# starreeze/drin

Measured on AMD Instinct MI355X. Metric: mention x candidate pairs scored/sec, higher is better.
Workload: dtype bf16x3; 1 GPU; wikimel-shaped scoring forward: 100-cand (+1 answer slot), D=768, R=2048, L=128, P=49, T=64 token-level entity text; parallelism=dp1 (mentions sharded, no collective)

## Files before the change

### drin_amd/_lib.py

```python
from __future__ import annotations

import ctypes as C
import os
from typing import Optional

_HERE = os.path.dirname(os.path.abspath(__file__))
LIB_PATH = os.environ.get("DRIN_LIB_PATH") or os.path.join(_HERE, "libdrin_hip.so")
MAX_LAYERS = 8
ABI_VERSION = 12

OK, E_SHAPE, E_NULL, E_ALIGN, E_WORKSPACE, E_HIP, E_UNSUPPORTED, E_INDEX = 0, -1, -2, -3, -4, -5, -6, -7
PREC_F32, PREC_BF16X3, PREC_BF16X3_ALL, PREC_BF16X3_IF16 = 0, 1, 3, 5
ROW_ACT = {"none": 0, "relu": 1, "gelu": 2}
FEAT_F32, FEAT_BF16 = 0, 1
CACHE_F32, CACHE_MIXED_F16 = 0, 1
CACHE_FORMATS = {"f32": CACHE_F32, "mixed_f16": CACHE_MIXED_F16}
ACTIVATIONS = {"gelu": 1, "sigmoid": 2, "relu": 3, "tanh": 4, "silu": 5}

fp = C.POINTER(C.c_float)
ip = C.POINTER(C.c_int64)


class DrinConfigC(C.Structure):
    _fields_ = [
        ("batch", C.c_int32), ("num_candidates", C.c_int32), ("embed_dim", C.c_int32), ("image_dim", C.c_int32),
        ("mention_tokens", C.c_int32), ("image_regions", C.c_int32), ("mention_objects", C.c_int32),
        ("entity_objects", C.c_int32), ("entity_tokens", C.c_int32), ("mention_object_inner", C.c_int32),
        ("entity_image_inner", C.c_int32), ("entity_object_inner", C.c_int32), ("num_layers", C.c_int32),
        ("dynamic_edges", C.c_int32), ("edge_enabled", C.c_float * 4), ("layer_norm_eps", C.c_float),
        ("cosine_eps", C.c_float), ("miei_eps", C.c_float), ("clip_scale", C.c_float), ("precision", C.c_int32),
        ("num_entities", C.c_int32), ("vector_edges", C.c_int32), ("feature_dtype", C.c_int32),
        ("vertex_activation", C.c_int32), ("edge_activation", C.c_int32), ("cache_format", C.c_int32),
    ]


class DrinBatchC(C.Structure):
    _fields_ = [
        ("mention_text", C.c_void_p), ("mention_start", C.c_void_p), ("mention_end", C.c_void_p),
        ("mention_image", C.c_void_p), ("mention_object", C.c_void_p), ("mention_object_score", C.c_void_p),
        ("entity_text", C.c_void_p), ("entity_text_mask", C.c_void_p), ("entity_image", C.c_void_p),
        ("entity_object", C.c_void_p), ("entity_object_score", C.c_void_p), ("miet_similarity", C.c_void_p),
        ("mtei_similarity", C.c_void_p), ("entity_index", C.c_void_p), ("entity_text_cls", C.c_void_p),
        ("index_status", C.c_void_p),
    ]


class DrinLayerParamsC(C.Structure):
    _fields_ = [(n, C.c_void_p) for n in ("w_h", "b_h", "w_u", "b_u", "w_v", "b_v", "ln_weight", "ln_bias", "w_m", "b_m")]


class DrinParamsC(C.Structure):
    _fields_ = [(n, C.c_void_p) for n in (
        "w_mention_text", "b_mention_text", "w_entity_text", "b_entity_text",
        "w_mention_image", "b_mention_image", "w_entity_image", "b_entity_image")] + [("layer", DrinLayerParamsC * MAX_LAYERS)]


class DrinParamGradsC(C.Structure):
    _fields_ = DrinParamsC._fields_


class DrinInputGradsC(C.Structure):
    _fields_ = [(n, C.c_void_p) for n in (
        "mention_text", "mention_image", "mention_object", "mention_object_score", "entity_text", "entity_text_cls",
        "entity_image", "entity_object", "entity_object_score", "miet_similarity", "mtei_similarity", "scratch")] + [
        ("scratch_bytes", C.c_size_t)]


class DrinMelhiConfigC(C.Structure):
    _fields_ = [("batch", C.c_int32), ("num_candidates", C.c_int32), ("embed_dim", C.c_int32), ("image_dim", C.c_int32),
                ("mention_tokens", C.c_int32), ("image_regions", C.c_int32), ("precision", C.c_int32),
                ("cosine_eps", C.c_float), ("thres_tmim", C.c_float), ("thres_imie", C.c_float)]


class DrinMelhiBatchC(C.Structure):
    _fields_ = [(n, C.c_void_p) for n in (
        "mention_feature", "mention_mask", "start", "end", "mention_image", "entity_feature", "entity_image")]


MELHI_PARAMS = ("w_image_map_text", "b_image_map_text", "w_ih", "w_hh", "b_ih", "b_hh", "w_mention_final_map",
                "b_mention_final_map", "w_entity_final_map", "b_entity_final_map")


class DrinMelhiParamsC(C.Structure):
    _fields_ = [(n, C.c_void_p) for n in MELHI_PARAMS]


class DrinMelhiParamGradsC(C.Structure):
    _fields_ = DrinMelhiParamsC._fields_


class DrinGhmfcConfigC(C.Structure):
    _fields_ = [("batch", C.c_int32), ("num_candidates", C.c_int32), ("embed_dim", C.c_int32), ("image_dim", C.c_int32),
                ("mention_tokens", C.c_int32), ("image_regions", C.c_int32), ("num_heads", C.c_int32),
                ("entity_tokens", C.c_int32), ("precision", C.c_int32), ("layer_norm_eps", C.c_float), ("cosine_eps", C.c_float)]


class DrinGhmfcBatchC(C.Structure):
    _fields_ = [(n, C.c_void_p) for n in ("mention_feature", "mention_mask", "mention_image", "entity_feature", "entity_mask")]


GHMFC_CROSS_PARAMS = ("a2b_wq", "a2b_wk", "a2b_wv", "a2b_in_bias", "a2b_wo", "a2b_bo", "a2b_ffn_w", "a2b_ffn_b", "b2a_in_w",
                      "b2a_in_bias", "b2a_wo", "b2a_bo", "b2a_ffn_w", "b2a_ffn_b", "ln0_w", "ln0_b", "ln1_w", "ln1_b", "ln2_w",
                      "ln2_b", "ln3_w", "ln3_b")


class DrinGhmfcCrossParamsC(C.Structure):
    _fields_ = [(n, C.c_void_p) for n in GHMFC_CROSS_PARAMS]


class DrinGhmfcParamsC(C.Structure):
    _fields_ = [("t2v", DrinGhmfcCrossParamsC), ("v2t", DrinGhmfcCrossParamsC)] + [(n, C.c_void_p) for n in (
        "w_text_linear", "b_text_linear", "w_image_linear", "b_image_linear", "w_score_linear", "b_score_linear", "w_entity",
        "b_entity")]


class DrinGemmRouteC(C.Structure):
    _fields_ = [(n, C.c_int32) for n in ("launches", "family", "bm", "bn", "w_planes", "a_lo", "f16", "persist", "indexed", "accumulate",
                                         "ksplit", "splits")] + [(n, C.c_int64) for n in ("tiles", "whole_tiles", "tile0", "work_items")]


class DrinGemmProbeArgsC(C.Structure):
    _fields_ = [("struct_size", C.c_size_t), ("op", C.c_int32), ("precision", C.c_int32), ("accumulate", C.c_int32),
                ("row_tile_wgs", C.c_int32), ("row_tile_begin", C.c_int64), ("row_tile_end", C.c_int64), ("a", C.c_void_p),
                ("a_lo", C.c_void_p), ("lda", C.c_int64), ("b", C.c_void_p), ("b_hi", C.c_void_p), ("b_lo", C.c_void_p),
                ("ldb", C.c_int64), ("bias", C.c_void_p), ("y", C.c_void_p), ("ldy", C.c_int64), ("rows", C.c_int64),
                ("n_out", C.c_int32), ("k", C.c_int32), ("scratch", C.c_void_p), ("scratch_floats", C.c_size_t),
                ("a_index", C.c_void_p), ("row_scale", C.c_void_p), ("b_scale", C.c_void_p), ("route", DrinGemmRouteC)]


class DrinWgradProductC(C.Structure):
    _fields_ = [("dy", C.c_void_p), ("lddy", C.c_int64), ("x", C.c_void_p), ("ldx", C.c_int64), ("x_index", C.c_void_p), ("dw", C.c_void_p),
                ("lddw", C.c_int64), ("db", C.c_void_p), ("rows", C.c_int64), ("n_out", C.c_int32), ("k", C.c_int32)]


class DrinWgradProductRouteC(C.Structure):
    _fields_ = [(n, C.c_int32) for n in ("kernel", "slices", "in_place", "db_rode", "db_slices", "launch")] + [("rows_per_slice", C.c_int64)]


WGRAD_PROBE_MAX, WGRAD_ROUTE_LAUNCHES = 16, 8


class DrinWgradRouteC(C.Structure):
    _fields_ = [(n, C.c_int32) for n in ("gemm_launches", "colsum_launches", "sum_launches", "reduce_launches", "sum_dsts", "sum_segs",
                                         "nn_family", "nn_bm", "nn_bn", "nn_splits", "nn_wt_form", "nn_accumulate")] + [
        ("grid", C.c_int64 * WGRAD_ROUTE_LAUNCHES), ("product", DrinWgradProductRouteC * WGRAD_PROBE_MAX)]


class DrinWgradProbeArgsC(C.Structure):
    _fields_ = [("struct_size", C.c_size_t), ("op", C.c_int32), ("precision", C.c_int32), ("staged", C.c_int32), ("n_products", C.c_int32),
                ("layers_done_after", C.c_int32), ("accumulate", C.c_int32), ("wt_form", C.c_int32), ("reserved", C.c_int32),
                ("scratch", C.c_void_p), ("scratch_floats", C.c_size_t), ("wt", C.c_void_p), ("wt_floats", C.c_size_t),
                ("product", DrinWgradProductC * WGRAD_PROBE_MAX), ("route", DrinWgradRouteC)]


WGRAD_TN_GROUP, WGRAD_TN_F32_GROUP, WGRAD_TN, WGRAD_COLSUM_BATCH, WGRAD_PASS, WGRAD_NN = range(1, 7)
WGRAD_KERNEL = {0: "none", 1: "tn_bf16x3", 2: "tn_f32_small", 3: "tn_f32_large"}
WGRAD_WT_NONE, WGRAD_WT_F32_SCRATCH, WGRAD_WT_PLANES = range(3)
PROBE_GEMM_NT, PROBE_GEMM_NT_BF16X3, PROBE_GEMM_NT_BF16X3_P4, PROBE_GEMM_X3_PLANES, PROBE_GEMM_F16_PLANES, PROBE_TO_F16_SCALED = range(1, 7)
GEMM_FAMILY = {0: "none", 1: "bf16x3", 2: "bf16x3_p4", 3: "planes", 4: "planes_p4", 5: "f32", 6: "f32_gemv"}


class DrinTraceC(C.Structure):
    _fields_ = [(n, C.c_void_p * (MAX_LAYERS + 1)) for n in (
        "mention_text_vertex", "mention_image_vertex", "entity_text_vertex", "entity_image_vertex", "edges")]


EXPORTS = {
    "drin_version": (C.c_int, []),
    "drin_last_error": (C.c_char_p, []),
    "drin_build_info": (C.c_char_p, []),
    "drin_default_config": (C.c_int, [C.POINTER(DrinConfigC)]),
    "drin_host_selftest": (C.c_int, []),
    "drin_workspace_bytes": (C.c_size_t, [C.POINTER(DrinConfigC), C.c_int]),
    "drin_edges_fwd": (C.c_int, [C.POINTER(DrinConfigC), C.POINTER(DrinBatchC), C.c_void_p, C.c_void_p, C.c_void_p]),
    "drin_pool_fwd": (C.c_int, [C.POINTER(DrinConfigC), C.POINTER(DrinBatchC), C.c_void_p, C.c_void_p, C.c_void_p, C.c_void_p]),
    "drin_linear_fwd": (C.c_int, [C.c_void_p, C.c_void_p, C.c_void_p, C.c_void_p, C.c_int64, C.c_int32, C.c_int32, C.c_int32, C.c_void_p]),
    "drin_linear_bwd": (C.c_int, [C.c_void_p, C.c_void_p, C.c_void_p, C.c_void_p, C.c_void_p, C.c_void_p, C.c_int64, C.c_int32,
                                  C.c_int32, C.c_int32, C.c_void_p, C.c_size_t, C.c_void_p]),
    "drin_forward": (C.c_int, [C.POINTER(DrinConfigC), C.POINTER(DrinBatchC), C.POINTER(DrinParamsC), C.c_void_p,
                               C.c_size_t, C.c_void_p, C.c_int, C.POINTER(DrinTraceC), C.c_void_p]),
    "drin_forward_staged": (C.c_int, [C.POINTER(DrinConfigC), C.POINTER(DrinBatchC), C.POINTER(DrinParamsC), C.c_void_p,
                                      C.c_size_t, C.c_void_p, C.c_int, C.POINTER(DrinTraceC), C.c_void_p, C.c_void_p]),
    "drin_backward": (C.c_int, [C.POINTER(DrinConfigC), C.POINTER(DrinBatchC), C.POINTER(DrinParamsC), C.c_void_p,
                                C.c_size_t, C.c_void_p, C.POINTER(DrinParamGradsC), C.c_void_p]),
    "drin_backward_staged": (C.c_int, [C.POINTER(DrinConfigC), C.POINTER(DrinBatchC), C.POINTER(DrinParamsC), C.c_void_p,
                                       C.c_size_t, C.c_void_p, C.POINTER(DrinParamGradsC), C.c_void_p, C.c_void_p]),
    "drin_backward_ex": (C.c_int, [C.POINTER(DrinConfigC), C.POINTER(DrinBatchC), C.POINTER(DrinParamsC), C.c_void_p,
                                   C.c_size_t, C.c_void_p, C.POINTER(DrinParamGradsC), C.POINTER(DrinInputGradsC), C.c_void_p,
                                   C.c_void_p]),
    "drin_input_grad_scratch_bytes": (C.c_size_t, [C.POINTER(DrinConfigC)]),
    "drin_pool_bwd": (C.c_int, [C.POINTER(DrinConfigC), C.c_void_p, C.c_void_p, C.c_void_p, C.c_void_p, C.c_void_p]),
    "drin_fused_supported": (C.c_int, [C.POINTER(DrinConfigC)]),
    "drin_indexed_supported": (C.c_int, [C.POINTER(DrinConfigC)]),
    "drin_prepared_bytes": (C.c_size_t, [C.POINTER(DrinConfigC)]),
    "drin_fused_workspace_bytes": (C.c_size_t, [C.POINTER(DrinConfigC)]),
    "drin_workgroups_per_mention": (C.c_int32, [C.POINTER(DrinConfigC), C.c_int32]),
    "drin_index_status": (C.c_int, [C.c_void_p, C.c_void_p]),
    "drin_image_contraction_passes": (C.c_int32, [C.POINTER(DrinConfigC), C.c_int32]),
    "drin_image_contraction_side_tiles": (C.c_int32, [C.POINTER(DrinConfigC), C.c_int32]),
    "drin_prepare": (C.c_int, [C.POINTER(DrinConfigC), C.POINTER(DrinParamsC), C.c_void_p, C.c_size_t, C.c_void_p]),
    "drin_forward_prepared": (C.c_int, [C.POINTER(DrinConfigC), C.POINTER(DrinBatchC), C.POINTER(DrinParamsC), C.c_void_p,
                                        C.c_void_p, C.c_size_t, C.c_void_p, C.c_void_p]),
    "drin_entity_cache_bytes": (C.c_size_t, [C.POINTER(DrinConfigC)]),
    "drin_entity_cache_build_workspace_bytes": (C.c_size_t, [C.POINTER(DrinConfigC)]),
    "drin_cached_workspace_bytes": (C.c_size_t, [C.POINTER(DrinConfigC)]),
    "drin_build_entity_cache": (C.c_int, [C.POINTER(DrinConfigC), C.POINTER(DrinBatchC), C.POINTER(DrinParamsC), C.c_void_p,
                                          C.c_void_p, C.c_size_t, C.c_void_p, C.c_size_t, C.c_void_p]),
    "drin_forward_cached": (C.c_int, [C.POINTER(DrinConfigC), C.POINTER(DrinBatchC), C.POINTER(DrinParamsC), C.c_void_p,
                                      C.c_void_p, C.c_void_p, C.c_size_t, C.c_void_p, C.c_void_p]),
    "drin_split_planes": (C.c_int, [C.c_void_p, C.c_void_p, C.c_void_p, C.c_int64, C.c_void_p]),
    "drin_linear_planes_fwd": (C.c_int, [C.c_void_p, C.c_void_p, C.c_void_p, C.c_void_p, C.c_void_p, C.c_void_p,
                                         C.c_int64, C.c_int32, C.c_int32, C.c_void_p]),
    "drin_gemm_probe": (C.c_int, [C.POINTER(DrinGemmProbeArgsC), C.c_void_p]),
    "drin_wgrad_probe": (C.c_int, [C.POINTER(DrinWgradProbeArgsC), C.c_void_p]),
    "drin_loss_workspace_bytes": (C.c_size_t, [C.c_int32]),
    "drin_triplet_topk": (C.c_int, [C.c_void_p, C.c_void_p, C.c_int32, C.c_int32, C.c_float, C.POINTER(C.c_int32), C.c_int32,
                                    C.c_void_p, C.c_void_p, C.c_void_p, C.c_void_p, C.c_size_t, C.c_void_p]),
    "drin_adam_step": (C.c_int, [C.c_void_p, C.c_void_p, C.c_void_p, C.c_void_p, C.c_int64, C.c_float, C.c_float, C.c_float,
                                 C.c_float, C.c_float, C.c_float, C.c_void_p]),
    "drin_melhi_workspace_bytes": (C.c_size_t, [C.POINTER(DrinMelhiConfigC), C.c_int]),
    "drin_melhi_forward": (C.c_int, [C.POINTER(DrinMelhiConfigC), C.POINTER(DrinMelhiBatchC), C.POINTER(DrinMelhiParamsC), C.c_void_p,
                                     C.c_void_p, C.c_void_p, C.c_size_t, C.c_void_p, C.c_void_p]),
    "drin_melhi_backward": (C.c_int, [C.POINTER(DrinMelhiConfigC), C.POINTER(DrinMelhiBatchC), C.POINTER(DrinMelhiParamsC),
                                      C.c_void_p, C.c_void_p, C.c_void_p, C.c_size_t, C.c_void_p, C.POINTER(DrinMelhiParamGradsC),
                                      C.c_void_p]),
    "drin_ghmfc_workspace_bytes": (C.c_size_t, [C.POINTER(DrinGhmfcConfigC)]),
    "drin_ghmfc_forward": (C.c_int, [C.POINTER(DrinGhmfcConfigC), C.POINTER(DrinGhmfcBatchC), C.POINTER(DrinGhmfcParamsC), C.c_void_p,
                                     C.c_size_t, C.c_void_p, C.c_void_p, C.c_void_p]),
    "drin_attention": (C.c_int, [C.c_void_p, C.c_int64, C.c_void_p, C.c_int64, C.c_void_p, C.c_int64, C.c_void_p, C.c_void_p, C.c_int64,
                                 C.c_int32, C.c_int32, C.c_int32, C.c_int32, C.c_int32, C.c_void_p]),
    "drin_attention_train_fwd": (C.c_int, [C.c_void_p, C.c_int64, C.c_void_p, C.c_int64, C.c_void_p, C.c_int64, C.c_void_p, C.c_void_p,
                                           C.c_int64, C.c_void_p, C.c_int32, C.c_int32, C.c_int32, C.c_int32, C.c_int32, C.c_void_p]),
    "drin_attention_bwd": (C.c_int, [C.c_void_p, C.c_int64, C.c_void_p, C.c_int64, C.c_void_p, C.c_int64, C.c_void_p, C.c_void_p,
                                     C.c_int64, C.c_void_p, C.c_void_p, C.c_int64, C.c_void_p, C.c_int64, C.c_void_p, C.c_int64,
                                     C.c_void_p, C.c_int64, C.c_void_p, C.c_int32, C.c_int32, C.c_int32, C.c_int32, C.c_int32,
                                     C.c_void_p]),
    "drin_attention_dropout_fwd": (C.c_int, [C.c_void_p, C.c_int64, C.c_void_p, C.c_int64, C.c_void_p, C.c_int64, C.c_void_p, C.c_void_p,
                                             C.c_int64, C.c_void_p, C.c_int32, C.c_int32, C.c_int32, C.c_int32, C.c_int32, C.c_float,
                                             C.c_uint64, C.c_uint64, C.c_void_p]),
    "drin_attention_dropout_bwd": (C.c_int, [C.c_void_p, C.c_int64, C.c_void_p, C.c_int64, C.c_void_p, C.c_int64, C.c_void_p, C.c_void_p,
                                             C.c_int64, C.c_void_p, C.c_void_p, C.c_int64, C.c_void_p, C.c_int64, C.c_void_p, C.c_int64,
                                             C.c_void_p, C.c_int64, C.c_void_p, C.c_int32, C.c_int32, C.c_int32, C.c_int32, C.c_int32,
                                             C.c_float, C.c_uint64, C.c_uint64, C.c_void_p]),
    "drin_attention_dropout_keep": (C.c_int, [C.c_uint64, C.c_uint64, C.c_int32, C.c_int32, C.c_int32, C.c_int32, C.c_float, C.c_void_p]),
    "drin_attention_mfma_fwd": (C.c_int, [C.c_void_p, C.c_int64, C.c_void_p, C.c_int64, C.c_void_p, C.c_int64, C.c_void_p, C.c_void_p,
                                          C.c_int64, C.c_void_p, C.c_int32, C.c_int32, C.c_int32, C.c_int32, C.c_int32, C.c_float,
                                          C.c_uint64, C.c_uint64, C.c_void_p]),
    "drin_attention_mfma_bwd": (C.c_int, [C.c_void_p, C.c_int64, C.c_void_p, C.c_int64, C.c_void_p, C.c_int64, C.c_void_p, C.c_void_p,
                                          C.c_int64, C.c_void_p, C.c_void_p, C.c_int64, C.c_void_p, C.c_int64, C.c_void_p, C.c_int64,
                                          C.c_void_p, C.c_int64, C.c_void_p, C.c_int32, C.c_int32, C.c_int32, C.c_int32, C.c_int32,
                                          C.c_float, C.c_uint64, C.c_uint64, C.c_void_p]),
    "drin_layernorm_res_train_fwd": (C.c_int, [C.c_void_p, C.c_void_p, C.c_void_p, C.c_void_p, C.c_void_p, C.c_void_p, C.c_void_p,
                                               C.c_int64, C.c_int32, C.c_float, C.c_void_p]),
    "drin_layernorm_res_bwd_scratch_floats": (C.c_size_t, [C.c_int64, C.c_int32]),
    "drin_layernorm_res_bwd": (C.c_int, [C.c_void_p, C.c_void_p, C.c_void_p, C.c_void_p, C.c_void_p, C.c_void_p, C.c_void_p, C.c_void_p,
                                         C.c_void_p, C.c_void_p, C.c_size_t, C.c_int64, C.c_int32, C.c_void_p]),
    "drin_seq_max_train_fwd": (C.c_int, [C.c_void_p, C.c_void_p, C.c_void_p, C.c_int32, C.c_int32, C.c_int32, C.c_void_p]),
    "drin_seq_max_bwd": (C.c_int, [C.c_void_p, C.c_void_p, C.c_void_p, C.c_int32, C.c_int32, C.c_int32, C.c_void_p]),
    "drin_gate_mix_fwd": (C.c_int, [C.c_void_p, C.c_void_p, C.c_void_p, C.c_void_p, C.c_void_p, C.c_int32, C.c_int32, C.c_void_p]),
    "drin_gate_mix_bwd_scratch_floats": (C.c_size_t, [C.c_int32, C.c_int32]),
    "drin_gate_mix_bwd": (C.c_int, [C.c_void_p, C.c_void_p, C.c_void_p, C.c_void_p, C.c_void_p, C.c_void_p, C.c_void_p, C.c_void_p,
                                    C.c_void_p, C.c_void_p, C.c_size_t, C.c_int32, C.c_int32, C.c_void_p]),
    "drin_cosine_rows_fwd": (C.c_int, [C.c_void_p, C.c_void_p, C.c_void_p, C.c_int32, C.c_int32, C.c_int32, C.c_float, C.c_void_p]),
    "drin_cosine_rows_bwd": (C.c_int, [C.c_void_p, C.c_void_p, C.c_void_p, C.c_void_p, C.c_void_p, C.c_void_p, C.c_size_t, C.c_int32,
                                       C.c_int32, C.c_int32, C.c_float, C.c_void_p]),
    "drin_entity_token_mean": (C.c_int, [C.c_void_p, C.c_void_p, C.c_void_p, C.c_int64, C.c_int32, C.c_int32, C.c_void_p]),
    "drin_act_dropout_fwd": (C.c_int, [C.c_void_p, C.c_void_p, C.c_int64, C.c_int32, C.c_int32, C.c_float, C.c_uint64, C.c_uint64,
                                       C.c_void_p]),
    "drin_act_dropout_bwd": (C.c_int, [C.c_void_p, C.c_void_p, C.c_void_p, C.c_int64, C.c_int32, C.c_int32, C.c_float, C.c_uint64,
                                       C.c_uint64, C.c_void_p]),
    "drin_span_mean_fwd": (C.c_int, [C.c_void_p, C.c_void_p, C.c_void_p, C.c_void_p, C.c_int32, C.c_int32, C.c_int32, C.c_void_p]),
    "drin_span_mean_bwd": (C.c_int, [C.c_void_p, C.c_void_p, C.c_void_p, C.c_void_p, C.c_int32, C.c_int32, C.c_int32, C.c_void_p]),
    "drin_profile_begin": (C.c_int, [C.c_int]),
    "drin_profile_end": (C.c_int, [C.POINTER(C.c_double), C.POINTER(C.c_int64)]),
    "drin_kernel_class_name": (C.c_char_p, [C.c_int]),
}
KERNEL_CLASSES = 12


class DrinError(RuntimeError):
    def __init__(self, status: int, message: str):
        super().__init__(f"libdrin_hip status {status}: {message}")
        self.status = status


_lib: Optional[C.CDLL] = None


def load() -> C.CDLL:
    global _lib
    if _lib is not None:
        return _lib
    if not os.path.exists(LIB_PATH):
        raise ImportError(
            f"{LIB_PATH} is missing: the DRIN HIP path has no fallback. Build it with `python -m drin_amd.build`."
        )
    try:
        import torch
    except ImportError:
        pass
    lib = C.CDLL(LIB_PATH)
    for name, (res, args) in EXPORTS.items():
        fn = getattr(lib, name)
        fn.restype, fn.argtypes = res, args
    if lib.drin_version() != ABI_VERSION:
        raise ImportError(f"libdrin_hip ABI {lib.drin_version()} != binding {ABI_VERSION}; rebuild")
    _lib = lib
    return lib


def profile_begin(max_launches: int = 65536) -> None:
    check(load().drin_profile_begin(max_launches))


def profile_end() -> dict:
    ms = (C.c_double * KERNEL_CLASSES)()
    n = (C.c_int64 * KERNEL_CLASSES)()
    check(load().drin_profile_end(ms, n))
    lib = load()
    return {lib.drin_kernel_class_name(k).decode(): (ms[k], n[k]) for k in range(KERNEL_CLASSES)}


def check(status: int) -> None:
    if status != OK:
        raise DrinError(status, load().drin_last_error().decode())


def _ptr(t) -> C.c_void_p:
    return C.c_void_p(t.data_ptr()) if t is not None else C.c_void_p(0)


def _stream(device) -> C.c_void_p:
    import torch
    return C.c_void_p(torch.cuda.current_stream(device).cuda_stream)


def _scratch(pool: dict, device, stream_id: int, floats: int):
    import torch
    buf = pool.get((device, stream_id))
    if buf is None or buf.numel() < floats:
        buf = pool[(device, stream_id)] = torch.empty(max(floats, 1), dtype=torch.float32, device=device)
    return buf
```

### drin_amd/csrc/fused.h

```cpp
#pragma once
#include <hip/hip_runtime.h>
#include <stddef.h>
#include <stdint.h>
#include <string.h>

#include "../../include/drin_hip.h"
#include "layout.h"

namespace drin {

struct Prepared {
  size_t wcat1, bcat1, ecat, etmp, k_t, k_i, c_txt, c_img, cb_t, cb_i, total;
  size_t p_ctxt, p_cimg, p_wh2;
  size_t p_wmt, p_wmi, p_wcat1, p_ecat, p_wet, p_wei, p_wh1;
  size_t p_cimg_f16;
  size_t cimg_f16_scale;
  void build(const drin_config& c) {
    const size_t D = c.embed_dim, R = c.image_dim;
    Arena A;
    wcat1 = A.take(2 * D * D);
    bcat1 = A.take(2 * D);
    ecat = A.take(D * (D + R));
    etmp = A.take(D * (D + R));
    k_t = A.take(D);
    k_i = A.take(D);
    c_txt = A.take(D * D);
    c_img = A.take(D * R);
    cb_t = A.take(D);
    cb_i = A.take(D);
    p_ctxt = A.take(D * D);
    p_cimg = A.take(D * R);
    p_wh2 = A.take(D * D);
    p_wmt = A.take(D * D);
    p_wmi = A.take(D * R);
    p_wcat1 = A.take(2 * D * D);
    p_ecat = A.take(D * (D + R));
    p_wet = A.take(D * D);
    p_wei = A.take(D * R);
    p_wh1 = A.take(D * D);
    p_cimg_f16 = A.take(D * R / 2 + 2);
    cimg_f16_scale = A.take(2);
    total = A.total;
  }
};

int fused_supported(const drin_config* c);
int cached_chunks_per_mention(const drin_config& c);

struct StreamArgs {
  const void* entity_text;
  const int64_t* entity_mask;
  const void* entity_image;
  const void* entity_object;
  const float* entity_object_score;
  const int64_t* entity_index;
  int64_t num_entities;
  int32_t* index_status;
  const float* miet;
  const float* mtei;
  const float* span_mean;
  const void* mobj;
  const float* mscore;
  const float* fu;
  const float* q;
  const float* k_t;
  const float* k_i;
  float* xt_out;
  void* xt_hi;
  void* xt_lo;
  void* xi_hi;
  void* xi_lo;
  float* xi_scale;
  void* xi_f16;
  float* e0m;
  float* e1m;
  float* s_part;
  float* s_text;
  float* s_img;
  float* sig;
  int B, N, D4, R4, T, Km, Ke, chunks, ldq, ldfu, dynamic, bf16_features;
  int act_e;
  float mask[4];
  float cos_eps, miei_eps, clip;
};

struct PairArgs {
  const float* h_text;
  const float* h_image;
  const float* hm;
  const float* c_t;
  const float* c_i;
  const float* gamma;
  const float* beta;
  const float* e0m;
  const float* e1m;
  float* et1;
  void* et1_hi;
  void* et1_lo;
  float* s2_part;
  int B, N, D4, chunks, ldhm;
  int act_v;
  float ln_eps;
};

struct FinalArgs {
  const float* h2;
  const float* hm2;
  const float* b_h2;
  const float* gamma;
  const float* beta;
  const float* e1m;
  const float* mt2;
  float* scores;
  int B, N, D4, chunks;
  int act_v;
  float ln_eps, cos_eps;
};

template <class Args>
Args shaped_args(const drin_config& c) {
  Args a;
  memset(&a, 0, sizeof(a));
  a.B = c.batch, a.N = c.num_candidates, a.D4 = c.embed_dim / 4;
  return a;
}
template <class Args>
void set_vertex_fields(Args& a, const drin_config& c) {
  a.ln_eps = c.layer_norm_eps, a.act_v = vertex_act(&c);
}
template <class Args>
void set_edge_fields(Args& a, const drin_config& c) {
  a.R4 = c.image_dim / 4;
  a.Km = c.mention_objects;
  a.dynamic = c.dynamic_edges != 0;
  a.act_e = edge_act(&c);
  for (int k = 0; k < 4; ++k) a.mask[k] = c.edge_enabled[k];
  a.cos_eps = c.cosine_eps, a.miei_eps = c.miei_eps, a.clip = c.clip_scale;
}

size_t entity_stream_lds_bytes(const StreamArgs& a);
int launch_entity_stream(const StreamArgs& a, hipStream_t st);
int launch_reduce_stream_partials(const float* part, float* s_text, float* s_img, float* sig, int B, int D, int R,
                                  int chunks, hipStream_t st);
int launch_mention_input1(const float* T, const float* T2, const float* sig, const float* b_et, const float* b_ei,
                          const float* v0, float* out, int B, int D, int N, hipStream_t st);
int launch_pair_layer1(const PairArgs& a, hipStream_t st);
int launch_mention_input2(const float* part, const float* mt1, float* out, int B, int D, int N, int chunks,
                          hipStream_t st);
int launch_pair_final(const FinalArgs& a, hipStream_t st);

struct GemmScratch {
  float* p = nullptr;
  size_t floats = 0;
};
int run_folded_head(const drin_config* cfg, const drin_batch* b, const drin_params* params, const float* prepared, const Prepared& P,
                    bool weight_planes, float* span_mean, float* mimg, float* vm0, float* hmfu, GemmScratch mention_sk, hipStream_t st);
int run_folded_mention_finish(const drin_config* cfg, const drin_params* params, const float* prepared, const Prepared& P,
                              bool weight_planes, float* vm1, float* hm2, GemmScratch mention_sk, hipStream_t st);
int run_folded_tail(const drin_config* cfg, const drin_params* params, const float* prepared, const Prepared& P, int chunks,
                    const float* s2_part, const float* vm1, float* agg2, float* mt2, const float* hm2, const float* e1m, float* h2,
                    const float* et1, const void* et1_hi, bool weight_planes, GemmScratch mention_sk, GemmScratch pair_sk,
                    float* scores, hipStream_t st);
}
```

### drin_amd/csrc/fused_forward.hip

```cpp
#include <string.h>

#include "fused.h"
#include "internal.h"
#include "layout.h"

namespace drin {

constexpr int kMixedMinCandidates = 64;

struct FusedLayout {
  size_t span_mean, mimg, vm0, hmfu, q, e0m, e1m, xt, s_part, s_text, s_img, sig, tm, tm2, agg1, vm1, hm2, h_text, h_image,
      et1, s2_part, agg2, mt2, p_xt, p_xi, p_et1, xi_scale, splitk, splitk_floats, pair_splitk, pair_splitk_floats, total;
  int chunks;
  void build(const drin_config& c) {
    const size_t B = c.batch, N = c.num_candidates, D = c.embed_dim, R = c.image_dim, M = B * N;
    chunks = (int)(B >= 2048 ? (N + 127) / 128 : B >= 1024 ? (N + 47) / 48 : (N + 15) / 16);
    Arena A;
    span_mean = A.take(B * D);
    mimg = A.take(B * R);
    vm0 = A.take(2 * B * D);
    hmfu = A.take(2 * B * 2 * D);
    q = A.take(2 * B * (D + R));
    e0m = A.take(4 * M);
    e1m = A.take(4 * M);
    xt = A.take(c.entity_tokens > 0 ? M * D : 0);
    s_part = A.take(B * chunks * (2 * D + 2 * R + 4));
    s_text = A.take(2 * B * D);
    s_img = A.take(2 * B * R);
    sig = A.take(4 * B);
    tm = A.take(2 * B * D);
    tm2 = A.take(2 * B * D);
    agg1 = A.take(2 * B * D);
    vm1 = A.take(2 * B * D);
    hm2 = A.take(2 * B * D);
    h_text = A.take(M * D);
    h_image = A.take(M * D);
    et1 = A.take(M * D);
    s2_part = A.take(B * chunks * 2 * D);
    agg2 = A.take(B * D);
    mt2 = A.take(B * D);
    const bool planes = c.precision == DRIN_PREC_BF16X3 || c.precision == DRIN_PREC_BF16X3_ALL || c.precision == DRIN_PREC_BF16X3_IF16;
    p_xt = A.take(planes ? M * D : 0);
    p_xi = A.take(!planes ? 0 : c.num_entities > 0 ? M * R : c.precision == DRIN_PREC_BF16X3_IF16 ? M * R / 2 : 0);
    p_et1 = A.take(planes ? M * D : 0);
    xi_scale = A.take(c.precision == DRIN_PREC_BF16X3_IF16 ? M : 0);
    splitk_floats = 2 * B <= (size_t)kSmallSplitkMaxRows ? small_splitk_floats(2 * B, D + R) : 0;
    if (planes && splitk_floats < tail_split_floor_floats()) splitk_floats = tail_split_floor_floats();
    splitk = A.take(splitk_floats);
    pair_splitk_floats = planes ? drin::pair_splitk_floats(M, D) : 0;
    pair_splitk = A.take(pair_splitk_floats);
    total = A.total;
  }
};

int fused_layout_selfcheck(const drin_config& c) {
  const size_t B = c.batch, M = B * c.num_candidates, D = c.embed_dim, R = c.image_dim;
  FusedLayout L;
  L.build(c);
  const size_t ch = (size_t)L.chunks, planes = c.precision != DRIN_PREC_F32;
  const Region ws[] = {
      {"span_mean", L.span_mean, B * D}, {"mimg", L.mimg, B * R}, {"vm0", L.vm0, 2 * B * D}, {"hmfu", L.hmfu, 4 * B * D},
      {"q", L.q, 2 * B * (D + R)}, {"e0m", L.e0m, 4 * M}, {"e1m", L.e1m, 4 * M}, {"xt", L.xt, c.entity_tokens > 0 ? M * D : 0},
      {"s_part", L.s_part, B * ch * (2 * D + 2 * R + 4)}, {"s_text", L.s_text, 2 * B * D}, {"s_img", L.s_img, 2 * B * R},
      {"sig", L.sig, 4 * B}, {"tm", L.tm, 2 * B * D}, {"tm2", L.tm2, 2 * B * D}, {"agg1", L.agg1, 2 * B * D}, {"vm1", L.vm1, 2 * B * D},
      {"hm2", L.hm2, 2 * B * D}, {"h_text", L.h_text, M * D}, {"h_image", L.h_image, M * D}, {"et1", L.et1, M * D},
      {"s2_part", L.s2_part, B * ch * 2 * D}, {"agg2", L.agg2, B * D}, {"mt2", L.mt2, B * D}, {"p_xt", L.p_xt, planes * M * D},
      {"p_xi", L.p_xi, !planes ? 0 : c.num_entities > 0 ? M * R : c.precision == DRIN_PREC_BF16X3_IF16 ? M * R / 2 : 0},
      {"p_et1", L.p_et1, planes * M * D}, {"xi_scale", L.xi_scale, c.precision == DRIN_PREC_BF16X3_IF16 ? M : 0},
      {"splitk", L.splitk, L.splitk_floats}, {"pair_splitk", L.pair_splitk, L.pair_splitk_floats}};
  DRIN_TRY(regions_hold("FusedLayout", ws, (int)(sizeof(ws) / sizeof(ws[0])), L.total));
  Prepared P;
  P.build(c);
  const Region pr[] = {
      {"wcat1", P.wcat1, 2 * D * D}, {"bcat1", P.bcat1, 2 * D}, {"ecat", P.ecat, D * (D + R)}, {"etmp", P.etmp, D * (D + R)},
      {"k_t", P.k_t, D}, {"k_i", P.k_i, D}, {"c_txt", P.c_txt, D * D}, {"c_img", P.c_img, D * R}, {"cb_t", P.cb_t, D}, {"cb_i", P.cb_i, D},
      {"p_ctxt", P.p_ctxt, D * D}, {"p_cimg", P.p_cimg, D * R}, {"p_wh2", P.p_wh2, D * D}, {"p_wmt", P.p_wmt, D * D},
      {"p_wmi", P.p_wmi, D * R}, {"p_wcat1", P.p_wcat1, 2 * D * D}, {"p_ecat", P.p_ecat, D * (D + R)}, {"p_wet", P.p_wet, D * D},
      {"p_wei", P.p_wei, D * R}, {"p_wh1", P.p_wh1, D * D}, {"p_cimg_f16", P.p_cimg_f16, D * R / 2}, {"cimg_f16_scale", P.cimg_f16_scale, 2}};
  return regions_hold("Prepared", pr, (int)(sizeof(pr) / sizeof(pr[0])), P.total);
}

static bool if16_gate(const drin_config* c, bool indexed) {
  const int64_t M = (int64_t)c->batch * c->num_candidates;
  return c->precision == DRIN_PREC_BF16X3_IF16 && !indexed && c->feature_dtype == DRIN_FEAT_F32 &&
         c->num_candidates >= kMixedMinCandidates && c->embed_dim == 768 && c->image_dim == 2048 &&
         cdiv(M, 256) * cdiv(c->embed_dim, 256) >= 128;
}

#ifndef DRIN_SIDE_WGS
#define DRIN_SIDE_WGS 64
#endif
#ifndef DRIN_SIDE_PERMILLE
#define DRIN_SIDE_PERMILLE 900
#endif
#ifndef DRIN_SIDE_MIN_TILES
#define DRIN_SIDE_MIN_TILES 1200
#endif
constexpr int kSideWgs = DRIN_SIDE_WGS;
constexpr int kSidePermille = DRIN_SIDE_PERMILLE;
constexpr int64_t kSideMinTiles = DRIN_SIDE_MIN_TILES;
#ifdef DRIN_SIDE_PROBE
static int g_probe_wgs = kSideWgs, g_probe_permille = kSidePermille;
extern "C" __attribute__((visibility("default"))) void drin_probe_side_plan(int wgs, int permille) { g_probe_wgs = wgs, g_probe_permille = permille; }
#endif
struct SidePlan {
  int64_t S = 0;
  int G = 0;
};
static SidePlan image_side_plan(const drin_config* c, bool indexed, bool capturing) {
  SidePlan plan;
  int wgs = kSideWgs, permille = kSidePermille;
#ifdef DRIN_SIDE_PROBE
  wgs = g_probe_wgs, permille = g_probe_permille;
#endif
  const bool split = c->precision == DRIN_PREC_BF16X3 || c->precision == DRIN_PREC_BF16X3_ALL || c->precision == DRIN_PREC_BF16X3_IF16;
  if (capturing || indexed || !split || if16_gate(c, indexed) || wgs <= 0 || permille <= 0) return plan;
  const int D = c->embed_dim, R = c->image_dim;
  if ((D % 32) || (R % 32) || c->batch <= 0) return plan;
  const int64_t M = (int64_t)c->batch * c->num_candidates;
  const int64_t nx = cdiv(D, 256), row_tiles = cdiv(M, 256), tiles = row_tiles * nx;
  if (tiles < 192 || tiles < kSideMinTiles || tiles > ((int64_t)1 << 28)) return plan;
  FusedLayout L;
  L.build(*c);
  const int64_t whole_rows = gemm_p4_whole_tiles(tiles, R, L.splitk_floats > 0, L.splitk_floats) / nx;
  int64_t S = (row_tiles * permille + 500) / 1000;
  S = S < whole_rows ? S : whole_rows;
  S = S < row_tiles - 1 ? S : row_tiles - 1;
  if (S <= 0) return plan;
  plan.S = S;
  plan.G = (int)(wgs < S * nx ? wgs : S * nx);
  return plan;
}

struct SideJoin {
  SideLane* lane = nullptr;
  hipStream_t st = nullptr;
  int join() {
    if (!lane) return DRIN_OK;
    const hipError_t e = hipStreamWaitEvent(st, lane->join, 0);
    lane = nullptr;
    return e == hipSuccess ? DRIN_OK : hip_fail(e, "hipStreamWaitEvent(side stream)");
  }
  ~SideJoin() { (void)join(); }
};

int fused_supported(const drin_config* c) {
  if (c->num_layers != 2) {
    set_error("fused path: built for num_layers == 2 (got %d); use drin_forward", c->num_layers);
    return DRIN_E_UNSUPPORTED;
  }
  if (c->vector_edges) {
    set_error("fused path: vector edge features (model.py:112-116) run on the layer-by-layer path; use drin_forward");
    return DRIN_E_UNSUPPORTED;
  }
  if (c->mention_object_inner > 1 || c->entity_object_inner > 1 || c->entity_image_inner > 1) {
    set_error("fused path: inner feature dims > 1 need the pooled path of drin_forward");
    return DRIN_E_UNSUPPORTED;
  }
  const bool tiny = c->embed_dim <= 256 && c->image_dim <= 256;
  const bool full = c->embed_dim <= 768 && c->image_dim <= 2048;
  if (!tiny && !full) {
    set_error("fused path: D=%d R=%d outside the built instantiations", c->embed_dim, c->image_dim);
    return DRIN_E_UNSUPPORTED;
  }
  return DRIN_OK;
}

}

using namespace drin;

extern "C" {

int drin_split_planes(const float* x, void* hi, void* lo, int64_t n, void* stream) {
  DRIN_BIND_DEVICE(stream, x, "drin_split_planes");
  if (!x || !hi || !lo) {
    set_error("drin_split_planes: NULL argument");
    return DRIN_E_NULL;
  }
  return launch_split_planes(x, hi, lo, n, (hipStream_t)stream);
}

int drin_linear_planes_fwd(const void* x_hi, const void* x_lo, const void* w_hi, const void* w_lo, const float* bias,
                           float* y, int64_t rows, int32_t n_out, int32_t k, void* stream) {
  DRIN_BIND_DEVICE(stream, y, "drin_linear_planes_fwd");
  if (!x_hi || !w_hi || !w_lo || !y) {
    set_error("drin_linear_planes_fwd: NULL argument");
    return DRIN_E_NULL;
  }
  return launch_gemm_x3_planes(x_hi, x_lo, k, w_hi, w_lo, k, bias, y, n_out, rows, n_out, k, (hipStream_t)stream);
}

int drin_fused_supported(const drin_config* cfg) {
  DRIN_TRY(validate_config(cfg));
  return fused_supported(cfg);
}

size_t drin_prepared_bytes(const drin_config* cfg) {
  if (validate_config(cfg) != DRIN_OK || fused_supported(cfg) != DRIN_OK) return 0;
  Prepared P;
  P.build(*cfg);
  return P.total * sizeof(float);
}

int drin_prepare(const drin_config* cfg, const drin_params* params, void* prepared, size_t prepared_bytes,
                 void* stream) {
  DRIN_BIND_DEVICE(stream, prepared, "drin_prepare");
  RoctxRange range("drin_prepare");
  DRIN_TRY(validate_config(cfg));
  DRIN_TRY(fused_supported(cfg));
  if (!params || !prepared) {
    set_error("drin_prepare: NULL argument");
    return DRIN_E_NULL;
  }
  Prepared P;
  P.build(*cfg);
  if (prepared_bytes < P.total * sizeof(float) || !aligned16(prepared)) {
    set_error("drin_prepare: buffer has %zu bytes (needs %zu) or is not 16-byte aligned", prepared_bytes,
              P.total * sizeof(float));
    return DRIN_E_WORKSPACE;
  }
  hipStream_t st = (hipStream_t)stream;
  float* pb = (float*)prepared;
  const int D = cfg->embed_dim, R = cfg->image_dim;
  const drin_layer_params& L1 = params->layer[0];
  const int F32 = DRIN_PREC_F32;
  auto copy = [&](float* dst, const float* src, size_t n) -> int {
    hipError_t e = hipMemcpyAsync(dst, src, n * sizeof(float), hipMemcpyDeviceToDevice, st);
    return e == hipSuccess ? DRIN_OK : hip_fail(e, "hipMemcpyAsync(prepare)");
  };
  DRIN_TRY(copy(pb + P.wcat1, L1.w_h, (size_t)D * D));
  DRIN_TRY(copy(pb + P.wcat1 + (size_t)D * D, L1.w_u, (size_t)D * D));
  {
    hipError_t e = hipMemsetAsync(pb + P.bcat1, 0, D * sizeof(float), st);
    if (e != hipSuccess) return hip_fail(e, "hipMemsetAsync(prepare)");
  }
  DRIN_TRY(copy(pb + P.bcat1 + D, L1.b_u, D));
  DRIN_TRY(launch_gemm_nn(L1.w_v, D, params->w_entity_text, D, pb + P.etmp, D + R, D, D, D, false, F32, st));
  DRIN_TRY(launch_gemm_nn(L1.w_v, D, params->w_entity_image, R, pb + P.etmp + D, D + R, D, R, D, false, F32, st));
  DRIN_TRY(launch_transpose(pb + P.etmp, pb + P.ecat, D, D + R, st));
  DRIN_TRY(launch_gemm_nt(params->b_entity_text, D, L1.w_v, D, L1.b_v, pb + P.k_t, D, 1, D, D, false, F32, st));
  DRIN_TRY(launch_gemm_nt(params->b_entity_image, D, L1.w_v, D, L1.b_v, pb + P.k_i, D, 1, D, D, false, F32, st));
  DRIN_TRY(launch_gemm_nn(L1.w_h, D, params->w_entity_text, D, pb + P.c_txt, D, D, D, D, false, F32, st));
  DRIN_TRY(launch_gemm_nn(L1.w_h, D, params->w_entity_image, R, pb + P.c_img, R, D, R, D, false, F32, st));
  DRIN_TRY(launch_gemm_nt(params->b_entity_text, D, L1.w_h, D, L1.b_h, pb + P.cb_t, D, 1, D, D, false, F32, st));
  DRIN_TRY(launch_gemm_nt(params->b_entity_image, D, L1.w_h, D, L1.b_h, pb + P.cb_i, D, 1, D, D, false, F32, st));
  {
    const size_t dd = (size_t)D * D, dr = (size_t)D * R;
    __bf16* q = reinterpret_cast<__bf16*>(pb + P.p_ctxt);
    DRIN_TRY(launch_split_planes(pb + P.c_txt, q, q + dd, dd, st));
    q = reinterpret_cast<__bf16*>(pb + P.p_cimg);
    DRIN_TRY(launch_split_planes(pb + P.c_img, q, q + dr, dr, st));
    DRIN_TRY(launch_to_f16_scaled(pb + P.c_img, pb + P.p_cimg_f16, (int64_t)dr, pb + P.cimg_f16_scale, st));
    q = reinterpret_cast<__bf16*>(pb + P.p_wh2);
    DRIN_TRY(launch_split_planes(params->layer[1].w_h, q, q + dd, dd, st));
    struct { size_t off; const float* w; size_t n; } extra[] = {
        {P.p_wmt, params->w_mention_text, dd},  {P.p_wmi, params->w_mention_image, dr},
        {P.p_wcat1, pb + P.wcat1, 2 * dd},      {P.p_ecat, pb + P.ecat, dd + dr},
        {P.p_wet, params->w_entity_text, dd},   {P.p_wei, params->w_entity_image, dr},
        {P.p_wh1, L1.w_h, dd}};
    for (const auto& e : extra) {
      q = reinterpret_cast<__bf16*>(pb + e.off);
      DRIN_TRY(launch_split_planes(e.w, q, q + e.n, e.n, st));
    }
  }
  return DRIN_OK;
}

}

namespace drin {

static int folded_precision(const drin_config* c) { return c->precision == DRIN_PREC_BF16X3_IF16 ? (int)DRIN_PREC_BF16X3 : c->precision; }

int run_folded_head(const drin_config* cfg, const drin_batch* b, const drin_params* params, const float* pb, const Prepared& P,
                    bool weight_planes, float* span_mean, float* mimg, float* vm0, float* hmfu, GemmScratch sk, hipStream_t st) {
  const int B = cfg->batch, D = cfg->embed_dim, R = cfg->image_dim, prec = folded_precision(cfg);
  auto wp = [&](size_t plane_off) -> const float* { return weight_planes ? pb + plane_off : nullptr; };
  if (cfg->feature_dtype == DRIN_FEAT_BF16) {
    DRIN_TRY(launch_span_mean_bf16(b->mention_text, b->mention_start, b->mention_end, span_mean, B, cfg->mention_tokens, D, st));
    DRIN_TRY(launch_axis_mean_bf16(b->mention_image, mimg, B, cfg->image_regions, R, st));
  } else {
    DRIN_TRY(launch_span_mean(b->mention_text, b->mention_start, b->mention_end, span_mean, B, cfg->mention_tokens, D, st));
    DRIN_TRY(launch_axis_mean(b->mention_image, mimg, B, cfg->image_regions, R, st));
  }
  DRIN_TRY(launch_gemm_nt_pair({span_mean, params->w_mention_text, params->b_mention_text, vm0, D, D, D, B, D, D, wp(P.p_wmt)},
                               {mimg, params->w_mention_image, params->b_mention_image, vm0 + (size_t)B * D, R, R, D, B, D, R, wp(P.p_wmi)},
                               prec, st, sk.p, sk.floats));
  return launch_gemm_nt(vm0, D, pb + P.wcat1, D, pb + P.bcat1, hmfu, 2 * D, 2 * (int64_t)B, 2 * D, D, false, prec, st, sk.p, sk.floats,
                        wp(P.p_wcat1));
}

int run_folded_mention_finish(const drin_config* cfg, const drin_params* params, const float* pb, const Prepared& P,
                              bool weight_planes, float* vm1, float* hm2, GemmScratch sk, hipStream_t st) {
  const int B = cfg->batch, D = cfg->embed_dim;
  const drin_layer_params& L1 = params->layer[0];
  DRIN_TRY(launch_layernorm_gelu(vm1, L1.ln_weight, L1.ln_bias, vm1, nullptr, nullptr, 2 * (int64_t)B, D, cfg->layer_norm_eps, st,
                                 vertex_act(cfg)));
  return launch_gemm_nt(vm1, D, params->layer[1].w_h, D, nullptr, hm2, D, 2 * (int64_t)B, D, D, false, folded_precision(cfg), st, sk.p,
                        sk.floats, weight_planes ? pb + P.p_wh2 : nullptr);
}

int run_folded_tail(const drin_config* cfg, const drin_params* params, const float* pb, const Prepared& P, int chunks,
                    const float* s2_part, const float* vm1, float* agg2, float* mt2, const float* hm2, const float* e1m, float* h2,
                    const float* et1, const void* et1_hi, bool weight_planes, GemmScratch sk, GemmScratch pair_sk, float* scores,
                    hipStream_t st) {
  const int B = cfg->batch, N = cfg->num_candidates, D = cfg->embed_dim, prec = folded_precision(cfg);
  const int64_t M = (int64_t)B * N;
  const drin_layer_params& L2 = params->layer[1];
  DRIN_TRY(launch_mention_input2(s2_part, vm1, agg2, B, D, N, chunks, st));
  DRIN_TRY(launch_gemm_nt(agg2, D, L2.w_h, D, L2.b_h, mt2, D, B, D, D, false, prec, st, sk.p, sk.floats,
                          weight_planes ? pb + P.p_wh2 : nullptr));
  DRIN_TRY(launch_layernorm_gelu(mt2, L2.ln_weight, L2.ln_bias, mt2, nullptr, nullptr, B, D, cfg->layer_norm_eps, st, vertex_act(cfg)));
  if (et1_hi) {
    const __bf16* e1 = static_cast<const __bf16*>(et1_hi);
    const __bf16* w2 = reinterpret_cast<const __bf16*>(pb + P.p_wh2);
    DRIN_TRY(launch_gemm_x3_planes(e1, e1 + (size_t)M * D, D, w2, w2 + (size_t)D * D, D, nullptr, h2, D, M, D, D, st, pair_sk.p,
                                   pair_sk.floats));
  } else {
    DRIN_TRY(launch_gemm_nt(et1, D, L2.w_h, D, nullptr, h2, D, M, D, D, false, prec, st));
  }
  FinalArgs fa = shaped_args<FinalArgs>(*cfg);
  set_vertex_fields(fa, *cfg);
  fa.h2 = h2;
  fa.hm2 = hm2;
  fa.b_h2 = L2.b_h;
  fa.gamma = L2.ln_weight;
  fa.beta = L2.ln_bias;
  fa.e1m = e1m;
  fa.mt2 = mt2;
  fa.scores = scores;
  fa.chunks = chunks;
  fa.cos_eps = cfg->cosine_eps;
  return launch_pair_final(fa, st);
}

static int forward_prepared_on_stream(const drin_config* cfg, const drin_batch* b, const drin_params* params, const void* prepared,
                                      void* workspace, float* scores, hipStream_t st) {
  FusedLayout L;
  L.build(*cfg);
  Prepared P;
  P.build(*cfg);
  float* ws = (float*)workspace;
  const float* pb = (const float*)prepared;
  const int B = cfg->batch, N = cfg->num_candidates, D = cfg->embed_dim, R = cfg->image_dim;
  const int64_t M = (int64_t)B * N;
  if (B == 0) return DRIN_OK;
  const int prec = folded_precision(cfg);
  const bool dyn = cfg->dynamic_edges != 0;
  const bool tokens = cfg->entity_tokens > 0;
  const bool planes = (prec == DRIN_PREC_BF16X3 || prec == DRIN_PREC_BF16X3_ALL) && (D % 32 == 0) && (R % 32 == 0);
  const bool indexed = b->entity_index != nullptr;
  const bool xi_planes = planes && indexed;
  const bool if16 = if16_gate(cfg, indexed) && gemm_f16_planes_fits(ws + L.p_xi, R, pb + P.p_cimg_f16, R, ws + L.h_image, D, M, D, R);
  hipStreamCaptureStatus capture = hipStreamCaptureStatusNone;
  if (hipStreamIsCapturing(st, &capture) != hipSuccess) {
    (void)hipGetLastError();
    capture = hipStreamCaptureStatusActive;
  }
  SidePlan side = image_side_plan(cfg, indexed, capture != hipStreamCaptureStatusNone);
  if (!aligned16(b->entity_image) || !aligned16(ws + L.h_image) || !b->entity_image) side = SidePlan();
  if (b->entity_text_cls) {
    set_error("drin_forward_prepared: entity_text_cls (text pooled ahead of time) is a form of the training entry points");
    return DRIN_E_UNSUPPORTED;
  }
  if (indexed && cfg->num_entities <= 0) {
    set_error("drin_forward_prepared: entity_index given but cfg.num_entities = %d", cfg->num_entities);
    return DRIN_E_SHAPE;
  }
  if (indexed && !planes) {
    set_error("drin_forward_prepared: entity_index needs the split-bf16 precision (the stream kernel gathers the "
              "GEMM operands as planes); gather on the caller side for DRIN_PREC_F32");
    return DRIN_E_UNSUPPORTED;
  }
  const bool bf16_feat = cfg->feature_dtype == DRIN_FEAT_BF16;
  if (bf16_feat && !planes) {
    set_error("drin_forward_prepared: bf16 features need the split-bf16 precision (DRIN_PREC_BF16X3) and D, R multiples of 32");
    return DRIN_E_UNSUPPORTED;
  }
  __bf16* xt_hi = reinterpret_cast<__bf16*>(ws + L.p_xt);
  __bf16* xi_hi = reinterpret_cast<__bf16*>(ws + L.p_xi);
  __bf16* e1_hi = reinterpret_cast<__bf16*>(ws + L.p_et1);
  const size_t MD = (size_t)M * D, MR = (size_t)M * R;
  const drin_layer_params& L1 = params->layer[0];

  auto wp = [&](size_t plane_off) -> const float* { return planes ? pb + plane_off : nullptr; };
  const GemmScratch msk{L.splitk_floats ? ws + L.splitk : nullptr, L.splitk_floats};
  float* vm0 = ws + L.vm0;
  float* hmfu = ws + L.hmfu;
  const bool xt_exact = bf16_feat && !tokens;
  const GemmScratch psk = L.pair_splitk_floats ? GemmScratch{ws + L.pair_splitk, L.pair_splitk_floats} : msk;
  auto image_rows_product = [&](hipStream_t on, RowTiles rows) -> int {
    const __bf16* ci = reinterpret_cast<const __bf16*>(pb + P.p_cimg);
    if (bf16_feat)
      return launch_gemm_x3_planes(b->entity_image, nullptr, R, ci, ci + (size_t)D * R, R, nullptr, ws + L.h_image, D, M, D, R, on, psk.p,
                                   psk.floats, rows);
    return launch_gemm_nt_bf16x3_p4((const float*)b->entity_image, R, ci, ci + (size_t)D * R, R, nullptr, ws + L.h_image, D, M, D, R, on, false,
                                    aligned16(psk.p) ? psk.p : nullptr, psk.floats, rows);
  };
  SideJoin side_join;
  if (side.S > 0) {
    SideLane* lane = nullptr;
    DRIN_TRY(side_lane(&lane));
    std::lock_guard<std::mutex> order(lane->order);
    hipError_t e = hipEventRecord(lane->fork, st);
    if (e == hipSuccess) e = hipStreamWaitEvent(lane->stream, lane->fork, 0);
    if (e != hipSuccess) return hip_fail(e, "fork to the side stream");
    const int rc = image_rows_product(lane->stream, RowTiles{0, side.S, side.G});
    e = hipEventRecord(lane->join, lane->stream);
    side_join.lane = lane, side_join.st = st;
    if (rc != DRIN_OK) return rc;
    if (e != hipSuccess) return hip_fail(e, "hipEventRecord(side stream)");
  }
  DRIN_TRY(run_folded_head(cfg, b, params, pb, P, planes, ws + L.span_mean, ws + L.mimg, vm0, hmfu, msk, st));
  if (dyn)
    DRIN_TRY(launch_gemm_nt(hmfu + D, 2 * D, pb + P.ecat, D, nullptr, ws + L.q, D + R, 2 * (int64_t)B, D + R, D, false, prec, st, msk.p,
                            msk.floats, wp(P.p_ecat)));
  StreamArgs sa = shaped_args<StreamArgs>(*cfg);
  set_edge_fields(sa, *cfg);
  sa.entity_text = b->entity_text;
  sa.entity_mask = b->entity_text_mask;
  sa.entity_image = b->entity_image;
  sa.entity_object = b->entity_object;
  sa.entity_object_score = b->entity_object_score;
  sa.entity_index = b->entity_index;
  sa.num_entities = cfg->num_entities;
  sa.index_status = b->index_status;
  sa.miet = b->miet_similarity;
  sa.mtei = b->mtei_similarity;
  sa.span_mean = ws + L.span_mean;
  sa.mobj = b->mention_object;
  sa.mscore = b->mention_object_score;
  sa.fu = hmfu + D;
  sa.ldfu = 2 * D;
  sa.q = ws + L.q;
  sa.ldq = D + R;
  sa.k_t = pb + P.k_t;
  sa.k_i = pb + P.k_i;
  sa.xt_out = planes ? nullptr : ws + L.xt;
  if (planes) {
    sa.xt_hi = xt_hi;
    sa.xt_lo = xt_exact ? nullptr : xt_hi + MD;
    if (xi_planes) {
      sa.xi_hi = xi_hi;
      sa.xi_lo = bf16_feat ? nullptr : xi_hi + MR;
    }
  }
  sa.xi_scale = if16 ? ws + L.xi_scale : nullptr;
  sa.xi_f16 = if16 ? static_cast<void*>(xi_hi) : nullptr;
  sa.e0m = ws + L.e0m;
  sa.e1m = ws + L.e1m;
  sa.s_part = ws + L.s_part;
  sa.T = cfg->entity_tokens;
  sa.Ke = cfg->entity_objects;
  sa.chunks = L.chunks;
  sa.bf16_features = bf16_feat ? 1 : 0;
  sa.s_text = ws + L.s_text;
  sa.s_img = ws + L.s_img;
  sa.sig = ws + L.sig;
  DRIN_TRY(launch_entity_stream(sa, st));
  if (L.chunks > 1)
    DRIN_TRY(launch_reduce_stream_partials(ws + L.s_part, ws + L.s_text, ws + L.s_img, ws + L.sig, B, D, R, L.chunks, st));
  DRIN_TRY(launch_gemm_nt_pair({ws + L.s_text, params->w_entity_text, nullptr, ws + L.tm, D, D, D, 2 * (int64_t)B, D, D, wp(P.p_wet)},
                               {ws + L.s_img, params->w_entity_image, nullptr, ws + L.tm2, R, R, D, 2 * (int64_t)B, D, R,
                                wp(P.p_wei)},
                               prec, st, msk.p, msk.floats));
  DRIN_TRY(launch_mention_input1(ws + L.tm, ws + L.tm2, ws + L.sig, params->b_entity_text, params->b_entity_image, vm0, ws + L.agg1, B, D, N, st));
  float* vm1 = ws + L.vm1;
  DRIN_TRY(launch_gemm_nt(ws + L.agg1, D, L1.w_h, D, L1.b_h, vm1, D, 2 * (int64_t)B, D, D, false, prec, st, msk.p, msk.floats, wp(P.p_wh1)));
  DRIN_TRY(run_folded_mention_finish(cfg, params, pb, P, planes, vm1, ws + L.hm2, msk, st));
  if (planes) {
    const __bf16* ct = reinterpret_cast<const __bf16*>(pb + P.p_ctxt);
    const __bf16* ci = reinterpret_cast<const __bf16*>(pb + P.p_cimg);
    DRIN_TRY(launch_gemm_x3_planes(xt_hi, xt_exact ? nullptr : xt_hi + MD, D, ct, ct + (size_t)D * D, D, nullptr, ws + L.h_text, D, M, D,
                                   D, st, psk.p, psk.floats));
    if (if16)
      DRIN_TRY(launch_gemm_f16_planes(xi_hi, R, pb + P.p_cimg_f16, R, ws + L.xi_scale, pb + P.cimg_f16_scale, ws + L.h_image, D, M, D, R,
                                      st, psk.p, psk.floats));
    else if (xi_planes)
      DRIN_TRY(launch_gemm_x3_planes(xi_hi, bf16_feat ? nullptr : xi_hi + MR, R, ci, ci + (size_t)D * R, R, nullptr, ws + L.h_image, D, M,
                                     D, R, st, psk.p, psk.floats));
    else if (side.S > 0) {
      DRIN_TRY(side_join.join());
      DRIN_TRY(image_rows_product(st, RowTiles{side.S, -1, 0}));
    } else if (bf16_feat)
      DRIN_TRY(launch_gemm_x3_planes(b->entity_image, nullptr, R, ci, ci + (size_t)D * R, R, nullptr, ws + L.h_image, D, M, D, R, st, psk.p,
                                     psk.floats));
    else
      DRIN_TRY(launch_gemm_nt_bf16x3(b->entity_image, R, pb + P.c_img, R, nullptr, ws + L.h_image, D, M, D, R, st, ci, ci + (size_t)D * R,
                                     false, psk.p, psk.floats));
  } else {
    const float* x_t = tokens ? ws + L.xt : b->entity_text;
    DRIN_TRY(launch_gemm_nt(x_t, D, pb + P.c_txt, D, nullptr, ws + L.h_text, D, M, D, D, false, prec, st));
    DRIN_TRY(launch_gemm_nt(b->entity_image, R, pb + P.c_img, R, nullptr, ws + L.h_image, D, M, D, R, false, prec, st));
  }
  PairArgs pa = shaped_args<PairArgs>(*cfg);
  set_vertex_fields(pa, *cfg);
  pa.h_text = ws + L.h_text;
  pa.h_image = ws + L.h_image;
  pa.hm = hmfu;
  pa.ldhm = 2 * D;
  pa.c_t = pb + P.cb_t;
  pa.c_i = pb + P.cb_i;
  pa.gamma = L1.ln_weight;
  pa.beta = L1.ln_bias;
  pa.e0m = ws + L.e0m;
  pa.e1m = ws + L.e1m;
  pa.et1 = planes ? nullptr : ws + L.et1;
  if (planes) {
    pa.et1_hi = e1_hi;
    pa.et1_lo = e1_hi + MD;
  }
  pa.s2_part = ws + L.s2_part;
  pa.chunks = L.chunks;
  DRIN_TRY(launch_pair_layer1(pa, st));
  return run_folded_tail(cfg, params, pb, P, L.chunks, ws + L.s2_part, vm1, ws + L.agg2, ws + L.mt2, ws + L.hm2, ws + L.e1m, ws + L.h_text,
                         planes ? nullptr : ws + L.et1, planes ? e1_hi : nullptr, planes, msk, psk, scores, st);
}

}

extern "C" {

int32_t drin_workgroups_per_mention(const drin_config* cfg, int32_t cached) {
  if (validate_config(cfg) != DRIN_OK || fused_supported(cfg) != DRIN_OK) return 0;
  if (cached) return cached_chunks_per_mention(*cfg);
  FusedLayout L;
  L.build(*cfg);
  return L.chunks;
}

int32_t drin_image_contraction_side_tiles(const drin_config* cfg, int32_t indexed) {
  if (validate_config(cfg) != DRIN_OK || fused_supported(cfg) != DRIN_OK) return 0;
  return (int32_t)image_side_plan(cfg, indexed != 0, false).S;
}

int32_t drin_image_contraction_passes(const drin_config* cfg, int32_t indexed) {
  if (validate_config(cfg) != DRIN_OK || fused_supported(cfg) != DRIN_OK) return 0;
  if (cfg->precision == DRIN_PREC_F32) return 0;
  if (if16_gate(cfg, indexed != 0)) return 1;
  return cfg->feature_dtype == DRIN_FEAT_BF16 ? 2 : 3;
}

int drin_index_status(int32_t* index_status, void* stream) {
  if (!index_status) {
    set_error("drin_index_status: NULL argument");
    return DRIN_E_NULL;
  }
  DRIN_BIND_DEVICE(stream, index_status, "drin_index_status");
  int32_t w[4] = {0, 0, 0, 0};
  hipError_t e = hipMemcpyAsync(w, index_status, sizeof(w), hipMemcpyDeviceToHost, (hipStream_t)stream);
  if (e == hipSuccess) e = hipStreamSynchronize((hipStream_t)stream);
  if (e != hipSuccess) return hip_fail(e, "drin_index_status");
  if (w[0] == 0) return DRIN_OK;
  e = hipMemsetAsync(index_status, 0, sizeof(w), (hipStream_t)stream);
  if (e != hipSuccess) return hip_fail(e, "drin_index_status(reset)");
  const long long value = (long long)(((uint64_t)(uint32_t)w[3] << 32) | (uint32_t)w[2]);
  set_error("entity_index out of range: candidate row %lld at pair %d (b * N + n) is outside the entity tables - the row was clamped "
            "and a WRONG entity scored; drin/data.py:87-93 raises IndexError here", value, (int)w[1]);
  return DRIN_E_INDEX;
}

size_t drin_fused_workspace_bytes(const drin_config* cfg) {
  if (validate_config(cfg) != DRIN_OK || fused_supported(cfg) != DRIN_OK) return 0;
  FusedLayout L;
  L.build(*cfg);
  return L.total * sizeof(float);
}

int drin_forward_prepared(const drin_config* cfg, const drin_batch* b, const drin_params* params, const void* prepared,
                          void* workspace, size_t workspace_bytes, float* scores, void* stream) {
  DRIN_BIND_DEVICE(stream, workspace, "drin_forward_prepared");
  RoctxRange range("drin_forward_prepared");
  DRIN_TRY(validate_config(cfg));
  DRIN_TRY(fused_supported(cfg));
  if (!b || !params || !prepared || !workspace || !scores) {
    set_error("drin_forward_prepared: NULL argument");
    return DRIN_E_NULL;
  }
  FusedLayout L;
  L.build(*cfg);
  if (workspace_bytes < L.total * sizeof(float) || !aligned16(workspace)) {
    set_error("drin_forward_prepared: workspace has %zu bytes (needs %zu) or is not 16-byte aligned", workspace_bytes,
              L.total * sizeof(float));
    return DRIN_E_WORKSPACE;
  }
  return forward_prepared_on_stream(cfg, b, params, prepared, workspace, scores, (hipStream_t)stream);
}

}
```

### drin_amd/csrc/fused_kernels.hip

```cpp
#include "device_utils.h"
#include "fused.h"
#include "internal.h"
#include "row_ops.h"

namespace drin {

template <int DV, int RV, bool TOKENS, bool EXACT, typename FT, bool XSCALE = false>
__global__ void __launch_bounds__(256, 2) k_entity_stream(const StreamArgs a) {
  extern __shared__ __attribute__((aligned(16))) float lds[];
  const FT* const f_text = static_cast<const FT*>(a.entity_text);
  const FT* const f_image = static_cast<const FT*>(a.entity_image);
  const FT* const f_object = static_cast<const FT*>(a.entity_object);
  const FT* const f_mobj = static_cast<const FT*>(a.mobj);
  const int D4 = EXACT ? DV * 64 : a.D4, R4 = EXACT ? RV * 64 : a.R4, D = D4 * 4, R = R4 * 4;
  constexpr bool RP = sizeof(FT) == 2 && (RV % 2) == 0;
  auto load_r = [&](const FT* row) -> Row<RV> {
    if constexpr (RP)
      return load_row_stream_pair<RV>(row, (int)(threadIdx.x & 63), R4);
    else
      return load_row_stream<RV>(row, (int)(threadIdx.x & 63), R4);
  };
  float* l_mobj = lds;
  float* l_q = l_mobj + a.Km * R;
  float* l_red = l_q + 2 * R;
  float* l_mt = l_red + 2 * D + 2 * R;
  float* l_small = l_mt + 3 * D;
  const int wave = threadIdx.x >> 6, lane = threadIdx.x & 63;
  const int64_t b = blockIdx.y;
  const int per = (a.N + a.chunks - 1) / a.chunks;
  const int n_begin = blockIdx.x * per, n_end = min(a.N, n_begin + per);
  const bool dyn = a.dynamic != 0;

  for (int i = threadIdx.x; i < a.Km * R4; i += 256) st4(l_mobj + i * 4, ld4(f_mobj + (b * a.Km) * R + i * 4));
  for (int i = threadIdx.x; i < D4; i += 256) st4(l_mt + i * 4, ld4(a.span_mean + b * D + i * 4));
  if (dyn) {
    for (int i = threadIdx.x; i < 2 * R4; i += 256) {
      const int which = i / R4, c4 = i - which * R4;
      st4(l_q + i * 4, ld4(a.q + ((int64_t)which * a.B + b) * a.ldq + D + c4 * 4));
    }
    for (int i = threadIdx.x; i < 2 * D4; i += 256) {
      const int which = i / D4, c4 = i - which * D4;
      st4(l_mt + D + i * 4, ld4(a.q + ((int64_t)which * a.B + b) * a.ldq + c4 * 4));
    }
  }
  __syncthreads();
  for (int i = wave; i < a.Km; i += 4) {
    float s = 0.f;
    for (int c4 = lane; c4 < R4; c4 += 64) {
      const float4 v = ld4(l_mobj + i * R + c4 * 4);
      s += dot4(v, v);
    }
    s = wave_sum(s);
    if (lane == 0) l_small[i] = fmaxf(sqrtf(s), a.cos_eps);
  }
  float m_t_norm;
  {
    const Row<DV> m_t = load_row<DV>(l_mt, lane, D4);
    m_t_norm = fmaxf(sqrtf(wave_sum(dot_rows<DV>(m_t, m_t))), a.cos_eps);
  }
  float kap_tt = 0.f, kap_ti = 0.f, kap_it = 0.f, kap_ii = 0.f;
  if (dyn) {
    const Row<DV> fu_t = load_row<DV>(a.fu + b * a.ldfu, lane, D4);
    const Row<DV> fu_i = load_row<DV>(a.fu + ((int64_t)a.B + b) * a.ldfu, lane, D4);
    const Row<DV> k_t = load_row<DV>(a.k_t, lane, D4), k_i = load_row<DV>(a.k_i, lane, D4);
    kap_tt = wave_sum(dot_rows<DV>(fu_t, k_t));
    kap_ti = wave_sum(dot_rows<DV>(fu_t, k_i));
    kap_it = wave_sum(dot_rows<DV>(fu_i, k_t));
    kap_ii = wave_sum(dot_rows<DV>(fu_i, k_i));
  }
  __syncthreads();

  Row<DV> S_tt = zero_row<DV>(), S_it = zero_row<DV>();
  Row<RV> S_ti = zero_row<RV>(), S_ii = zero_row<RV>();
  float sg_tt = 0.f, sg_ti = 0.f, sg_it = 0.f, sg_ii = 0.f;
  const float inv_d = 1.0f / (float)D;

  for (int n = n_begin + wave; n < n_end; n += 4) {
    const int64_t p = b * a.N + n;
    int64_t e = p;
    if (a.entity_index) {
      const int64_t raw = a.entity_index[p];
      e = raw < 0 ? 0 : (raw >= a.num_entities ? a.num_entities - 1 : raw);
      if (e != raw && lane == 0) report_bad_index(a.index_status, p, raw);
    }
    Row<DV> xt;
    float tt;
    if (TOKENS) {
      const int T = a.T;
      int cnt = 0;
      for (int t = lane; t < T; t += 64) cnt += (int)a.entity_mask[e * T + t];
      cnt = (int)wave_sum((float)cnt);
      int stop = cnt - 1;
      if (stop < 0) stop += T;
      stop = stop < 0 ? 0 : (stop > T ? T : stop);
      const FT* base = f_text + e * (int64_t)T * D;
      constexpr bool FLAT = sizeof(FT) == 2 && EXACT && DV == 3;
      const Row<DV> cls = load_row_stream<DV>(base, lane, D4);
      Row<DV> acc = zero_row<DV>();
      int t = 1;
      if constexpr (FLAT) {
        float f0[8], f1[8], f2[8];
#pragma unroll
        for (int i = 0; i < 8; ++i) f0[i] = f1[i] = f2[i] = 0.f;
        const char* flat = reinterpret_cast<const char*>(base) + (size_t)lane * 16;
        auto add8 = [](float (&f)[8], const u32x4_t v) {
#pragma unroll
          for (int i = 0; i < 4; ++i) {
            f[2 * i] += __builtin_bit_cast(float, v[i] << 16);
            f[2 * i + 1] += __builtin_bit_cast(float, v[i] & 0xffff0000u);
          }
        };
        for (; t + 8 <= stop; t += 8) {
          u32x4_t r[4][3];
#pragma unroll
          for (int u = 0; u < 4; ++u)
#pragma unroll
            for (int k = 0; k < 3; ++k) r[u][k] = ld16_stream(flat + (size_t)(t + 2 * u) * (2 * 768) + k * 1024);
#pragma unroll
          for (int u = 0; u < 4; ++u) {
            add8(f0, r[u][0]);
            add8(f1, r[u][1]);
            add8(f2, r[u][2]);
          }
        }
        for (; t + 2 <= stop; t += 2) {
          const u32x4_t r0 = ld16_stream(flat + (size_t)t * (2 * 768)), r1 = ld16_stream(flat + (size_t)t * (2 * 768) + 1024),
                        r2 = ld16_stream(flat + (size_t)t * (2 * 768) + 2048);
          add8(f0, r0);
          add8(f1, r1);
          add8(f2, r2);
        }
        float* scr = l_red + wave * 768;
#pragma unroll
        for (int i = 0; i < 8; ++i) {
          const float y1 = __shfl_xor(f1[i], 32), y2 = __shfl_xor(f2[i], 32);
          f0[i] += lane < 32 ? y1 : y2;
          f1[i] += y2;
        }
        st4(scr + 8 * lane, make_float4(f0[0], f0[1], f0[2], f0[3]));
        st4(scr + 8 * lane + 4, make_float4(f0[4], f0[5], f0[6], f0[7]));
        if (lane < 32) {
          st4(scr + 512 + 8 * lane, make_float4(f1[0], f1[1], f1[2], f1[3]));
          st4(scr + 512 + 8 * lane + 4, make_float4(f1[4], f1[5], f1[6], f1[7]));
        }
        __builtin_amdgcn_wave_barrier();
#pragma unroll
        for (int j = 0; j < DV; ++j) acc.v[j] = ld4(scr + 4 * (lane + 64 * j));
        __builtin_amdgcn_wave_barrier();
      } else if constexpr (sizeof(FT) == 2 && (EXACT || DV == 1)) {
        for (; t + 8 <= stop; t += 8) {
          Row<DV> r[8];
#pragma unroll
          for (int u = 0; u < 8; ++u) r[u] = load_row_stream<DV>(base + (int64_t)(t + u) * D, lane, D4);
#pragma unroll
          for (int u = 0; u < 8; ++u)
#pragma unroll
            for (int j = 0; j < DV; ++j) acc.v[j] = acc.v[j] + r[u].v[j];
        }
      }
      for (; t + 4 <= stop; t += 4) {
        const Row<DV> r0 = load_row_stream<DV>(base + (int64_t)t * D, lane, D4);
        const Row<DV> r1 = load_row_stream<DV>(base + (int64_t)(t + 1) * D, lane, D4);
        const Row<DV> r2 = load_row_stream<DV>(base + (int64_t)(t + 2) * D, lane, D4);
        const Row<DV> r3 = load_row_stream<DV>(base + (int64_t)(t + 3) * D, lane, D4);
#pragma unroll
        for (int j = 0; j < DV; ++j) acc.v[j] = (((acc.v[j] + r0.v[j]) + r1.v[j]) + r2.v[j]) + r3.v[j];
      }
      for (; t < stop; ++t) {
        const Row<DV> r0 = load_row_stream<DV>(base + (int64_t)t * D, lane, D4);
#pragma unroll
        for (int j = 0; j < DV; ++j) acc.v[j] = acc.v[j] + r0.v[j];
      }
      const float den = stop > 1 ? (float)(stop - 1) : 0.0f;
#pragma unroll
      for (int j = 0; j < DV; ++j)
        xt.v[j] = make_float4(acc.v[j].x / den, acc.v[j].y / den, acc.v[j].z / den, acc.v[j].w / den);
      if (a.xt_out) store_row<DV>(a.xt_out + p * D, xt, lane, D4);
      const float xy = wave_sum(dot_row_lds<DV>(cls, l_mt, lane, D4)), yy = wave_sum(dot_rows<DV>(cls, cls));
      tt = xy / (m_t_norm * fmaxf(sqrtf(yy), a.cos_eps));
    } else {
      xt = load_row_stream<DV>(f_text + e * D, lane, D4);
      const float xy = wave_sum(dot_row_lds<DV>(xt, l_mt, lane, D4)), yy = wave_sum(dot_rows<DV>(xt, xt));
      tt = xy / (m_t_norm * fmaxf(sqrtf(yy), a.cos_eps));
    }
    if (a.xt_hi) store_row_planes<DV>(a.xt_hi, a.xt_lo, p * D, xt, lane, D4);
    float sim = 0.f, wsum = 0.f;
    for (int j = 0; j < a.Ke; ++j) {
      const Row<RV> eo = load_r(f_object + (e * a.Ke + j) * R);
      const float ny = fmaxf(sqrtf(wave_sum(dot_rows<RV>(eo, eo))), a.cos_eps);
      const float es = a.entity_object_score[e * a.Ke + j];
      for (int i = 0; i < a.Km; ++i) {
        const float xy = wave_sum(dot_row_lds<RV, RP>(eo, l_mobj + i * R, lane, R4));
        const float w = a.mscore[b * a.Km + i] * es;
        sim += xy / (l_small[i] * ny) * w;
        wsum += w;
      }
    }
    const float ii = sim / (wsum + a.miei_eps);
    const Row<RV> xi = load_r(f_image + e * R);
    if (a.xi_hi) store_row_planes<RV, RP>(a.xi_hi, a.xi_lo, p * R, xi, lane, R4);
    if constexpr (XSCALE) {
      float m = 0.f;
#pragma unroll
      for (int j = 0; j < RV; ++j) m = fmaxf(m, fmaxf(fmaxf(fabsf(xi.v[j].x), fabsf(xi.v[j].y)), fmaxf(fabsf(xi.v[j].z), fabsf(xi.v[j].w))));
      const float sc = cache_field_scale(wave_max(m));
      if (lane == 0) a.xi_scale[p] = sc;
      store_row_f16_scaled<RV, RP>(a.xi_f16, p * R, xi, 1.0f / sc, lane);
    }
    const float e_tt = tt * a.mask[0];
    const float e_ti = (a.mtei[p] / a.clip) * a.mask[1];
    const float e_it = (a.miet[p] / a.clip) * a.mask[2];
    const float e_ii = ii * a.mask[3];
    float n_tt = e_tt, n_ti = e_ti, n_it = e_it, n_ii = e_ii;
    if (dyn) {
      const float d_tt = wave_sum(dot_row_lds<DV>(xt, l_mt + D, lane, D4));
      const float d_it = wave_sum(dot_row_lds<DV>(xt, l_mt + 2 * D, lane, D4));
      const float d_ti = wave_sum(dot_row_lds<RV, RP>(xi, l_q, lane, R4));
      const float d_ii = wave_sum(dot_row_lds<RV, RP>(xi, l_q + R, lane, R4));
      n_tt = edge_act_apply(a.act_e, (d_tt + kap_tt) * inv_d + e_tt);
      n_ti = edge_act_apply(a.act_e, (d_ti + kap_ti) * inv_d + e_ti);
      n_it = edge_act_apply(a.act_e, (d_it + kap_it) * inv_d + e_it);
      n_ii = edge_act_apply(a.act_e, (d_ii + kap_ii) * inv_d + e_ii);
    }
    if (lane == 0) {
      const int64_t M = (int64_t)a.B * a.N;
      a.e0m[p] = e_tt;
      a.e0m[M + p] = e_ti;
      a.e0m[2 * M + p] = e_it;
      a.e0m[3 * M + p] = e_ii;
      a.e1m[p] = n_tt * a.mask[0];
      a.e1m[M + p] = n_ti * a.mask[1];
      a.e1m[2 * M + p] = n_it * a.mask[2];
      a.e1m[3 * M + p] = n_ii * a.mask[3];
    }
    axpy_row<DV>(S_tt, e_tt, xt);
    axpy_row<DV>(S_it, e_it, xt);
    axpy_row<RV>(S_ti, e_ti, xi);
    axpy_row<RV>(S_ii, e_ii, xi);
    sg_tt += e_tt;
    sg_ti += e_ti;
    sg_it += e_it;
    sg_ii += e_ii;
  }

  for (int w = 0; w < 4; ++w) {
    __syncthreads();
    if (wave == w) {
#pragma unroll
      for (int j = 0; j < DV; ++j) {
        const int c4 = lane + 64 * j;
        if (c4 < D4) {
          float* p0 = l_red + c4 * 4;
          float* p1 = l_red + D + c4 * 4;
          st4(p0, w == 0 ? S_tt.v[j] : ld4(p0) + S_tt.v[j]);
          st4(p1, w == 0 ? S_it.v[j] : ld4(p1) + S_it.v[j]);
        }
      }
#pragma unroll
      for (int j = 0; j < RV; ++j) {
        const int c4 = row_col4<RP>(lane, j);
        if (c4 < R4) {
          float* p0 = l_red + 2 * D + c4 * 4;
          float* p1 = l_red + 2 * D + R + c4 * 4;
          st4(p0, w == 0 ? S_ti.v[j] : ld4(p0) + S_ti.v[j]);
          st4(p1, w == 0 ? S_ii.v[j] : ld4(p1) + S_ii.v[j]);
        }
      }
      if (lane == 0) {
        float* s4 = l_small + a.Km;
        s4[0] = (w == 0 ? 0.f : s4[0]) + sg_tt;
        s4[1] = (w == 0 ? 0.f : s4[1]) + sg_ti;
        s4[2] = (w == 0 ? 0.f : s4[2]) + sg_it;
        s4[3] = (w == 0 ? 0.f : s4[3]) + sg_ii;
      }
    }
  }
  __syncthreads();
  if (a.chunks == 1) {
    for (int i = threadIdx.x; i < 2 * D4; i += 256) {
      const int which = i / D4, c4 = i - which * D4;
      st4(a.s_text + ((int64_t)which * a.B + b) * D + c4 * 4, ld4(l_red + i * 4));
    }
    for (int i = threadIdx.x; i < 2 * R4; i += 256) {
      const int which = i / R4, c4 = i - which * R4;
      st4(a.s_img + ((int64_t)which * a.B + b) * R + c4 * 4, ld4(l_red + 2 * D + i * 4));
    }
    if (threadIdx.x < 4) a.sig[(int64_t)threadIdx.x * a.B + b] = l_small[a.Km + threadIdx.x];
    return;
  }
  float* out = a.s_part + (b * a.chunks + blockIdx.x) * (int64_t)(2 * D + 2 * R + 4);
  for (int i = threadIdx.x; i < (2 * D + 2 * R) / 4; i += 256) st4(out + i * 4, ld4(l_red + i * 4));
  if (threadIdx.x < 4) out[2 * D + 2 * R + threadIdx.x] = l_small[a.Km + threadIdx.x];
}

size_t entity_stream_lds_bytes(const StreamArgs& a) {
  const size_t D = (size_t)a.D4 * 4, R = (size_t)a.R4 * 4;
  return sizeof(float) * (a.Km * R + 2 * R + 2 * D + 2 * R + 3 * D + a.Km + 4);
}

template <int DV, int RV, bool TOKENS, bool EXACT, typename FT, bool XSCALE = false>
static int launch_stream_ft(const StreamArgs& a, hipStream_t st) {
  const size_t lds = entity_stream_lds_bytes(a);
  auto kern = k_entity_stream<DV, RV, TOKENS, EXACT, FT, XSCALE>;
  static DynLdsOptIn opt_in;
  if (lds > 48 * 1024)
    DRIN_TRY(ensure_dynamic_lds(opt_in, reinterpret_cast<const void*>(kern), (int)lds, "hipFuncSetAttribute(entity_stream)"));
  KernelTimer timer(DRIN_KC_STREAM, st);
  hipLaunchKernelGGL(kern, dim3((unsigned)a.chunks, (unsigned)a.B), dim3(256), lds, st, a);
  DRIN_CHECK_LAUNCH("k_entity_stream");
  return DRIN_OK;
}

template <int DV, int RV, bool TOKENS, bool EXACT>
static int launch_stream_t(const StreamArgs& a, hipStream_t st) {
  if (a.xi_scale != nullptr) {
    if constexpr (EXACT && DV == 3) {
      if (a.xi_f16 == nullptr) {
        set_error("entity_stream: xi_scale without xi_f16");
        return DRIN_E_NULL;
      }
      if (!a.bf16_features) return launch_stream_ft<DV, RV, TOKENS, EXACT, float, true>(a, st);
    }
    set_error("entity_stream: the scaled fp16 image plane is built for fp32-stored rows at D = 768, R = 2048");
    return DRIN_E_UNSUPPORTED;
  }
  return a.bf16_features ? launch_stream_ft<DV, RV, TOKENS, EXACT, __bf16>(a, st)
                         : launch_stream_ft<DV, RV, TOKENS, EXACT, float>(a, st);
}

int launch_entity_stream(const StreamArgs& a, hipStream_t st) {
  if (a.B <= 0) return DRIN_OK;
  if (a.B > 65535) {
    set_error("entity_stream: batch %d exceeds the grid limit; split the batch", a.B);
    return DRIN_E_SHAPE;
  }
  const bool tok = a.T > 0;
  if (a.D4 <= 64 && a.R4 <= 64)
    return tok ? launch_stream_t<1, 1, true, false>(a, st) : launch_stream_t<1, 1, false, false>(a, st);
  if (a.D4 == 192 && a.R4 == 512)
    return tok ? launch_stream_t<3, 8, true, true>(a, st) : launch_stream_t<3, 8, false, true>(a, st);
  if (a.D4 <= 192 && a.R4 <= 512)
    return tok ? launch_stream_t<3, 8, true, false>(a, st) : launch_stream_t<3, 8, false, false>(a, st);
  set_error("entity_stream: D=%d R=%d outside the built instantiations", a.D4 * 4, a.R4 * 4);
  return DRIN_E_UNSUPPORTED;
}

__global__ void __launch_bounds__(256) k_reduce_stream_partials(const float* __restrict__ part, float* __restrict__ s_text,
                                                                float* __restrict__ s_img, float* __restrict__ sig,
                                                                int B, int D, int R, int chunks) {
  const int64_t b = blockIdx.y;
  const int width = 2 * D + 2 * R + 4;
  const int i = (blockIdx.x * 256 + threadIdx.x) * 4;
  if (i >= width) return;
  const float* src = part + (b * chunks) * (int64_t)width + i;
  float4 s = make_float4(0.f, 0.f, 0.f, 0.f);
  int c = 0;
  for (; c + 4 <= chunks; c += 4) {
    const float4 v0 = ld4(src + (int64_t)c * width), v1 = ld4(src + (int64_t)(c + 1) * width);
    const float4 v2 = ld4(src + (int64_t)(c + 2) * width), v3 = ld4(src + (int64_t)(c + 3) * width);
    s = (((s + v0) + v1) + v2) + v3;
  }
  for (; c < chunks; ++c) s = s + ld4(src + (int64_t)c * width);
  if (i < D) {
    st4(s_text + b * D + i, s);
  } else if (i < 2 * D) {
    st4(s_text + ((int64_t)B + b) * D + (i - D), s);
  } else if (i < 2 * D + R) {
    st4(s_img + b * R + (i - 2 * D), s);
  } else if (i < 2 * D + 2 * R) {
    st4(s_img + ((int64_t)B + b) * R + (i - 2 * D - R), s);
  } else {
    sig[b] = s.x;
    sig[(int64_t)B + b] = s.y;
    sig[2 * (int64_t)B + b] = s.z;
    sig[3 * (int64_t)B + b] = s.w;
  }
}

int launch_reduce_stream_partials(const float* part, float* s_text, float* s_img, float* sig, int B, int D, int R,
                                  int chunks, hipStream_t st) {
  if (B <= 0) return DRIN_OK;
  KernelTimer timer(DRIN_KC_GCN, st);
  hipLaunchKernelGGL(k_reduce_stream_partials, dim3((unsigned)cdiv((2 * D + 2 * R + 4) / 4, 256), (unsigned)B), dim3(256), 0,
                     st, part, s_text, s_img, sig, B, D, R, chunks);
  DRIN_CHECK_LAUNCH("k_reduce_stream_partials");
  return DRIN_OK;
}

__global__ void __launch_bounds__(256) k_mention_input1(const float* __restrict__ T, const float* __restrict__ T2,
                                                        const float* __restrict__ sig,
                                                        const float* __restrict__ b_et, const float* __restrict__ b_ei,
                                                        const float* __restrict__ v0, float* __restrict__ out, int B,
                                                        int D, float inv_n) {
  const int64_t i = (int64_t)blockIdx.x * 256 + threadIdx.x;
  if (i >= 2 * (int64_t)B * D) return;
  const int d = (int)(i % D);
  const int64_t row = i / D;
  const int t = (int)(row / B);
  const int64_t b = row - (int64_t)t * B;
  const float sa = sig[(int64_t)(t == 0 ? 0 : 2) * B + b], sb = sig[(int64_t)(t == 0 ? 1 : 3) * B + b];
  out[i] = ((T[i] + T2[i]) + sa * b_et[d] + sb * b_ei[d]) * inv_n + v0[i];
}

int launch_mention_input1(const float* T, const float* T2, const float* sig, const float* b_et, const float* b_ei,
                          const float* v0, float* out, int B, int D, int N, hipStream_t st) {
  if (B <= 0) return DRIN_OK;
  KernelTimer timer(DRIN_KC_GCN, st);
  hipLaunchKernelGGL(k_mention_input1, dim3((unsigned)cdiv(2 * (int64_t)B * D, 256)), dim3(256), 0, st, T, T2, sig,
                     b_et, b_ei, v0, out, B, D, 1.0f / (float)N);
  DRIN_CHECK_LAUNCH("k_mention_input1");
  return DRIN_OK;
}

__global__ void __launch_bounds__(256) k_transpose(const float* __restrict__ in, float* __restrict__ out, int rows,
                                                   int cols) {
  __shared__ float tile[32][33];
  const int tx = threadIdx.x & 31, ty = threadIdx.x >> 5;
  const int r0 = blockIdx.y * 32, c0 = blockIdx.x * 32;
  for (int i = ty; i < 32; i += 8)
    if (r0 + i < rows && c0 + tx < cols) tile[i][tx] = in[(int64_t)(r0 + i) * cols + c0 + tx];
  __syncthreads();
  for (int i = ty; i < 32; i += 8)
    if (c0 + i < cols && r0 + tx < rows) out[(int64_t)(c0 + i) * rows + r0 + tx] = tile[tx][i];
}

int launch_transpose(const float* in, float* out, int rows, int cols, hipStream_t st) {
  if (rows <= 0 || cols <= 0) return DRIN_OK;
  KernelTimer timer(DRIN_KC_GCN, st);
  hipLaunchKernelGGL(k_transpose, dim3((unsigned)cdiv(cols, 32), (unsigned)cdiv(rows, 32)), dim3(256), 0, st, in, out,
                     rows, cols);
  DRIN_CHECK_LAUNCH("k_transpose");
  return DRIN_OK;
}

template <int DV, bool EXACT, bool GENERIC_ACT = false>
__global__ void __launch_bounds__(256) k_pair_layer1(const PairArgs a) {
  __shared__ __attribute__((aligned(16))) float l_red[2 * DV * 256];
  __shared__ __attribute__((aligned(16))) float l_const[6 * DV * 256];
  const int D4 = EXACT ? DV * 64 : a.D4, D = D4 * 4;
  const int wave = threadIdx.x >> 6, lane = threadIdx.x & 63;
  const int64_t b = blockIdx.y;
  const int64_t M = (int64_t)a.B * a.N;
  const int per = (a.N + a.chunks - 1) / a.chunks;
  const int n_begin = blockIdx.x * per, n_end = min(a.N, n_begin + per);
  constexpr int LD = DV * 256;
  {
    const float* src[6] = {a.hm + b * a.ldhm, a.hm + ((int64_t)a.B + b) * a.ldhm, a.c_t, a.c_i, a.gamma, a.beta};
#pragma unroll
    for (int v = 0; v < 6; ++v)
      for (int i = threadIdx.x; i < D4; i += 256) st4(l_const + v * LD + i * 4, ld4(src[v] + i * 4));
  }
  __syncthreads();
  const float *l_hm_t = l_const, *l_hm_i = l_const + LD, *l_ct = l_const + 2 * LD, *l_ci = l_const + 3 * LD;
  const float *l_gamma = l_const + 4 * LD, *l_beta = l_const + 5 * LD;
  Row<DV> S_t = zero_row<DV>(), S_i = zero_row<DV>();
  for (int n = n_begin + wave; n < n_end; n += 4) {
    const int64_t p = b * a.N + n;
    const Row<DV> ht = load_row_stream<DV>(a.h_text + p * D, lane, D4);
    const Row<DV> hi = load_row_stream<DV>(a.h_image + p * D, lane, D4);
    const float e_tt = a.e0m[p], e_ti = a.e0m[M + p], e_it = a.e0m[2 * M + p], e_ii = a.e0m[3 * M + p];
    const Row<DV> et1 = ln_gelu_row_lds<DV, GENERIC_ACT>(combine_rows_lds<DV>(ht, e_tt, l_hm_t, e_it, l_hm_i, l_ct, lane, D4),
                                                         l_gamma, l_beta, lane, D4, a.ln_eps, a.act_v);
    if (a.et1) store_row<DV>(a.et1 + p * D, et1, lane, D4);
    if (a.et1_hi) store_row_planes<DV>(a.et1_hi, a.et1_lo, p * D, et1, lane, D4);
    axpy_row_pk<DV>(S_t, a.e1m[p], et1);
    const Row<DV> ei1 = ln_gelu_row_lds<DV, GENERIC_ACT>(combine_rows_lds<DV>(hi, e_ti, l_hm_t, e_ii, l_hm_i, l_ci, lane, D4),
                                                         l_gamma, l_beta, lane, D4, a.ln_eps, a.act_v);
    axpy_row_pk<DV>(S_i, a.e1m[M + p], ei1);
  }
  for (int w = 0; w < 4; ++w) {
    __syncthreads();
    if (wave == w) {
#pragma unroll
      for (int j = 0; j < DV; ++j) {
        float* p0 = l_red + (j * 64 + lane) * 4;
        float* p1 = l_red + DV * 256 + (j * 64 + lane) * 4;
        st4(p0, w == 0 ? S_t.v[j] : ld4(p0) + S_t.v[j]);
        st4(p1, w == 0 ? S_i.v[j] : ld4(p1) + S_i.v[j]);
      }
    }
  }
  __syncthreads();
  float* out = a.s2_part + (b * a.chunks + blockIdx.x) * (int64_t)(2 * D);
  for (int i = threadIdx.x; i < 2 * D4; i += 256) {
    const int which = i / D4, c4 = i - which * D4;
    st4(out + which * D + c4 * 4, ld4(l_red + which * DV * 256 + c4 * 4));
  }
}

int launch_pair_layer1(const PairArgs& a, hipStream_t st) {
  if (a.B <= 0) return DRIN_OK;
  KernelTimer timer(DRIN_KC_GCN, st);
  if (a.act_v != DRIN_ACT_GELU && a.D4 <= 64)
    hipLaunchKernelGGL((k_pair_layer1<1, false, true>), dim3((unsigned)a.chunks, (unsigned)a.B), dim3(256), 0, st, a);
  else if (a.act_v != DRIN_ACT_GELU && a.D4 <= 192)
    hipLaunchKernelGGL((k_pair_layer1<3, false, true>), dim3((unsigned)a.chunks, (unsigned)a.B), dim3(256), 0, st, a);
  else if (a.D4 <= 64)
    hipLaunchKernelGGL((k_pair_layer1<1, false>), dim3((unsigned)a.chunks, (unsigned)a.B), dim3(256), 0, st, a);
  else if (a.D4 == 192)
    hipLaunchKernelGGL((k_pair_layer1<3, true>), dim3((unsigned)a.chunks, (unsigned)a.B), dim3(256), 0, st, a);
  else if (a.D4 < 192)
    hipLaunchKernelGGL((k_pair_layer1<3, false>), dim3((unsigned)a.chunks, (unsigned)a.B), dim3(256), 0, st, a);
  else {
    set_error("pair_layer1: D=%d outside the built instantiations", a.D4 * 4);
    return DRIN_E_UNSUPPORTED;
  }
  DRIN_CHECK_LAUNCH("k_pair_layer1");
  return DRIN_OK;
}

__global__ void __launch_bounds__(256) k_mention_input2(const float* __restrict__ part, const float* __restrict__ mt1,
                                                        float* __restrict__ out, int D, int chunks, float inv_n) {
  const int64_t b = blockIdx.y;
  const int d = blockIdx.x * 256 + threadIdx.x;
  if (d >= D) return;
  float st = 0.f, si = 0.f;
  for (int c = 0; c < chunks; ++c) {
    const float* p = part + (b * chunks + c) * (int64_t)(2 * D);
    st += p[d];
    si += p[D + d];
  }
  out[b * D + d] = (st * inv_n + si * inv_n) + mt1[b * D + d];
}

int launch_mention_input2(const float* part, const float* mt1, float* out, int B, int D, int N, int chunks,
                          hipStream_t st) {
  if (B <= 0) return DRIN_OK;
  KernelTimer timer(DRIN_KC_GCN, st);
  hipLaunchKernelGGL(k_mention_input2, dim3((unsigned)cdiv(D, 256), (unsigned)B), dim3(256), 0, st, part, mt1, out, D,
                     chunks, 1.0f / (float)N);
  DRIN_CHECK_LAUNCH("k_mention_input2");
  return DRIN_OK;
}

template <int DV, bool EXACT, bool GENERIC_ACT = false>
__global__ void __launch_bounds__(256) k_pair_final(const FinalArgs a) {
  __shared__ __attribute__((aligned(16))) float l_const[6 * DV * 256];
  const int D4 = EXACT ? DV * 64 : a.D4, D = D4 * 4;
  const int wave = threadIdx.x >> 6, lane = threadIdx.x & 63;
  const int64_t b = blockIdx.y;
  const int64_t M = (int64_t)a.B * a.N;
  const int per = (a.N + a.chunks - 1) / a.chunks;
  const int n_begin = blockIdx.x * per, n_end = min(a.N, n_begin + per);
  constexpr int LD = DV * 256;
  {
    const float* src[6] = {a.hm2 + b * D, a.hm2 + ((int64_t)a.B + b) * D, a.b_h2, a.gamma, a.beta, a.mt2 + b * D};
#pragma unroll
    for (int v = 0; v < 6; ++v)
      for (int i = threadIdx.x; i < D4; i += 256) st4(l_const + v * LD + i * 4, ld4(src[v] + i * 4));
  }
  __syncthreads();
  const Row<DV> mt2 = load_row<DV>(l_const + 5 * LD, lane, D4);
  const float xx = wave_sum(dot_rows<DV>(mt2, mt2));
  for (int n = n_begin + wave; n < n_end; n += 4) {
    const int64_t p = b * a.N + n;
    const Row<DV> h = load_row_stream<DV>(a.h2 + p * D, lane, D4);
    const Row<DV> et2 = ln_gelu_row_lds<DV, GENERIC_ACT>(
        combine_rows_lds<DV>(h, a.e1m[p], l_const, a.e1m[2 * M + p], l_const + LD, l_const + 2 * LD, lane, D4),
        l_const + 3 * LD, l_const + 4 * LD, lane, D4, a.ln_eps, a.act_v);
    const float xy = wave_sum(dot_rows_pk<DV>(mt2, et2));
    const float yy = wave_sum(dot_rows_pk<DV>(et2, et2));
    if (lane == 0) a.scores[p] = cosine_from_sums(xy, xx, yy, a.cos_eps);
  }
}

int launch_pair_final(const FinalArgs& a, hipStream_t st) {
  if (a.B <= 0) return DRIN_OK;
  KernelTimer timer(DRIN_KC_GCN, st);
  if (a.act_v != DRIN_ACT_GELU && a.D4 <= 64)
    hipLaunchKernelGGL((k_pair_final<1, false, true>), dim3((unsigned)a.chunks, (unsigned)a.B), dim3(256), 0, st, a);
  else if (a.act_v != DRIN_ACT_GELU && a.D4 <= 192)
    hipLaunchKernelGGL((k_pair_final<3, false, true>), dim3((unsigned)a.chunks, (unsigned)a.B), dim3(256), 0, st, a);
  else if (a.D4 <= 64)
    hipLaunchKernelGGL((k_pair_final<1, false>), dim3((unsigned)a.chunks, (unsigned)a.B), dim3(256), 0, st, a);
  else if (a.D4 == 192)
    hipLaunchKernelGGL((k_pair_final<3, true>), dim3((unsigned)a.chunks, (unsigned)a.B), dim3(256), 0, st, a);
  else if (a.D4 < 192)
    hipLaunchKernelGGL((k_pair_final<3, false>), dim3((unsigned)a.chunks, (unsigned)a.B), dim3(256), 0, st, a);
  else {
    set_error("pair_final: D=%d outside the built instantiations", a.D4 * 4);
    return DRIN_E_UNSUPPORTED;
  }
  DRIN_CHECK_LAUNCH("k_pair_final");
  return DRIN_OK;
}

}
```

### include/drin_hip.h

```cpp
#ifndef DRIN_HIP_H_
#define DRIN_HIP_H_

#include <stddef.h>
#include <stdint.h>

#ifdef __cplusplus
extern "C" {
#endif

#define DRIN_ABI_VERSION 12
#define DRIN_API __attribute__((visibility("default")))

typedef enum {
  DRIN_OK = 0,
  DRIN_E_SHAPE = -1,
  DRIN_E_NULL = -2,
  DRIN_E_ALIGN = -3,
  DRIN_E_WORKSPACE = -4,
  DRIN_E_HIP = -5,
  DRIN_E_UNSUPPORTED = -6,
  DRIN_E_INDEX = -7
} drin_status;

typedef enum {
  DRIN_PREC_F32 = 0,
  DRIN_PREC_BF16X3 = 1,
  DRIN_PREC_BF16X3_ALL = 3,
  DRIN_PREC_BF16X3_IF16 = 5
} drin_precision;

typedef struct {
  int32_t batch;
  int32_t num_candidates;
  int32_t embed_dim;
  int32_t image_dim;
  int32_t mention_tokens;
  int32_t image_regions;
  int32_t mention_objects;
  int32_t entity_objects;
  int32_t entity_tokens;
  int32_t mention_object_inner;
  int32_t entity_image_inner;
  int32_t entity_object_inner;
  int32_t num_layers;
  int32_t dynamic_edges;
  float edge_enabled[4];
  float layer_norm_eps;
  float cosine_eps;
  float miei_eps;
  float clip_scale;
  int32_t precision;
  int32_t num_entities;
  int32_t vector_edges;
  int32_t feature_dtype;
  int32_t vertex_activation;
  int32_t edge_activation;
  int32_t cache_format;
} drin_config;

typedef enum {
  DRIN_CACHE_F32 = 0,
  DRIN_CACHE_MIXED_F16 = 1
} drin_cache_format;

typedef enum {
  DRIN_ACT_DEFAULT = 0,
  DRIN_ACT_GELU = 1,
  DRIN_ACT_SIGMOID = 2,
  DRIN_ACT_RELU = 3,
  DRIN_ACT_TANH = 4,
  DRIN_ACT_SILU = 5
} drin_activation;

typedef enum {
  DRIN_FEAT_F32 = 0,
  DRIN_FEAT_BF16 = 1
} drin_feature_dtype;

typedef struct {
  const float* mention_text;
  const int64_t* mention_start;
  const int64_t* mention_end;
  const float* mention_image;
  const float* mention_object;
  const float* mention_object_score;
  const float* entity_text;
  const int64_t* entity_text_mask;
  const float* entity_image;
  const float* entity_object;
  const float* entity_object_score;
  const float* miet_similarity;
  const float* mtei_similarity;
  const int64_t* entity_index;
  const float* entity_text_cls;
  int32_t* index_status;
} drin_batch;

typedef struct {
  const float *w_h, *b_h, *w_u, *b_u, *w_v, *b_v, *ln_weight, *ln_bias;
  const float *w_m, *b_m;
} drin_layer_params;

#define DRIN_MAX_LAYERS 8

typedef struct {
  const float *w_mention_text, *b_mention_text;
  const float *w_entity_text, *b_entity_text;
  const float *w_mention_image, *b_mention_image;
  const float *w_entity_image, *b_entity_image;
  drin_layer_params layer[DRIN_MAX_LAYERS];
} drin_params;

typedef struct {
  float *w_mention_text, *b_mention_text, *w_entity_text, *b_entity_text;
  float *w_mention_image, *b_mention_image, *w_entity_image, *b_entity_image;
  struct { float *w_h, *b_h, *w_u, *b_u, *w_v, *b_v, *ln_weight, *ln_bias, *w_m, *b_m; } layer[DRIN_MAX_LAYERS];
} drin_param_grads;

typedef struct {
  float *mention_text, *mention_image, *mention_object, *mention_object_score;
  float *entity_text, *entity_text_cls, *entity_image, *entity_object, *entity_object_score;
  float *miet_similarity, *mtei_similarity;
  void* scratch;
  size_t scratch_bytes;
} drin_input_grads;

typedef struct {
  float* mention_text_vertex[DRIN_MAX_LAYERS + 1];
  float* mention_image_vertex[DRIN_MAX_LAYERS + 1];
  float* entity_text_vertex[DRIN_MAX_LAYERS + 1];
  float* entity_image_vertex[DRIN_MAX_LAYERS + 1];
  float* edges[DRIN_MAX_LAYERS + 1];
} drin_trace;

DRIN_API int drin_version(void);
DRIN_API const char* drin_last_error(void);
DRIN_API const char* drin_build_info(void);

DRIN_API int drin_default_config(drin_config* cfg);

DRIN_API int drin_host_selftest(void);

DRIN_API size_t drin_workspace_bytes(const drin_config* cfg, int for_training);


DRIN_API int drin_edges_fwd(const drin_config* cfg, const drin_batch* batch, float* edges, float* span_mean,
                   void* stream);

DRIN_API int drin_pool_fwd(const drin_config* cfg, const drin_batch* batch, float* pooled_entity_text,
                  float* pooled_mention_image, float* pooled_entity_image, void* stream);

DRIN_API int drin_linear_fwd(const float* x, const float* w, const float* bias, float* y, int64_t rows,
                    int32_t n_out, int32_t k, int32_t precision, void* stream);

DRIN_API int drin_linear_bwd(const float* x, const float* w, const float* dy, float* dx, float* dw, float* db,
                             int64_t rows, int32_t n_out, int32_t k, int32_t precision, float* scratch,
                             size_t scratch_floats, void* stream);

DRIN_API int drin_forward(const drin_config* cfg, const drin_batch* batch, const drin_params* params,
                 void* workspace, size_t workspace_bytes, float* scores, int keep_for_backward,
                 const drin_trace* trace, void* stream);

DRIN_API int drin_indexed_supported(const drin_config* cfg);

DRIN_API int drin_forward_staged(const drin_config* cfg, const drin_batch* batch, const drin_params* params,
                 void* workspace, size_t workspace_bytes, float* scores, int keep_for_backward,
                 const drin_trace* trace, void* params_ready_event, void* stream);

DRIN_API int drin_backward(const drin_config* cfg, const drin_batch* batch, const drin_params* params,
                  void* workspace, size_t workspace_bytes, const float* grad_scores,
                  const drin_param_grads* grads, void* stream);

DRIN_API int drin_backward_staged(const drin_config* cfg, const drin_batch* batch, const drin_params* params,
                  void* workspace, size_t workspace_bytes, const float* grad_scores,
                  const drin_param_grads* grads, void* layers_ready_event, void* stream);

DRIN_API int drin_backward_ex(const drin_config* cfg, const drin_batch* batch, const drin_params* params,
                              void* workspace, size_t workspace_bytes, const float* grad_scores,
                              const drin_param_grads* grads, const drin_input_grads* input_grads,
                              void* layers_ready_event, void* stream);
DRIN_API size_t drin_input_grad_scratch_bytes(const drin_config* cfg);

DRIN_API int drin_pool_bwd(const drin_config* cfg, const int64_t* entity_text_mask, const float* grad_pooled,
                           const float* grad_cls, void* grad_entity_text, void* stream);

DRIN_API int drin_fused_supported(const drin_config* cfg);
DRIN_API size_t drin_prepared_bytes(const drin_config* cfg);
DRIN_API size_t drin_fused_workspace_bytes(const drin_config* cfg);
DRIN_API int drin_prepare(const drin_config* cfg, const drin_params* params, void* prepared, size_t prepared_bytes,
                          void* stream);
DRIN_API int drin_forward_prepared(const drin_config* cfg, const drin_batch* batch, const drin_params* params,
                                   const void* prepared, void* workspace, size_t workspace_bytes, float* scores,
                                   void* stream);
DRIN_API int32_t drin_workgroups_per_mention(const drin_config* cfg, int32_t cached);

DRIN_API int32_t drin_image_contraction_passes(const drin_config* cfg, int32_t indexed);

DRIN_API int32_t drin_image_contraction_side_tiles(const drin_config* cfg, int32_t indexed);

DRIN_API int drin_index_status(int32_t* index_status, void* stream);

DRIN_API size_t drin_entity_cache_bytes(const drin_config* cfg);
DRIN_API size_t drin_entity_cache_build_workspace_bytes(const drin_config* cfg);
DRIN_API size_t drin_cached_workspace_bytes(const drin_config* cfg);
DRIN_API int drin_build_entity_cache(const drin_config* cfg, const drin_batch* tables, const drin_params* params,
                                     const void* prepared, void* cache, size_t cache_bytes, void* workspace,
                                     size_t workspace_bytes, void* stream);
DRIN_API int drin_forward_cached(const drin_config* cfg, const drin_batch* batch, const drin_params* params,
                                 const void* prepared, const void* cache, void* workspace, size_t workspace_bytes,
                                 float* scores, void* stream);

DRIN_API int drin_split_planes(const float* x, void* hi, void* lo, int64_t n, void* stream);
DRIN_API int drin_linear_planes_fwd(const void* x_hi, const void* x_lo, const void* w_hi, const void* w_lo,
                                    const float* bias, float* y, int64_t rows, int32_t n_out, int32_t k,
                                    void* stream);

enum drin_gemm_probe_op {
  DRIN_PROBE_GEMM_NT = 1,
  DRIN_PROBE_GEMM_NT_BF16X3 = 2,
  DRIN_PROBE_GEMM_NT_BF16X3_P4 = 3,
  DRIN_PROBE_GEMM_X3_PLANES = 4,
  DRIN_PROBE_GEMM_F16_PLANES = 5,
  DRIN_PROBE_TO_F16_SCALED = 6
};
enum drin_gemm_family {
  DRIN_GEMM_FAMILY_NONE = 0,
  DRIN_GEMM_FAMILY_BF16X3 = 1,
  DRIN_GEMM_FAMILY_BF16X3_P4 = 2,
  DRIN_GEMM_FAMILY_PLANES = 3,
  DRIN_GEMM_FAMILY_PLANES_P4 = 4,
  DRIN_GEMM_FAMILY_F32 = 5,
  DRIN_GEMM_FAMILY_F32_GEMV = 6
};
typedef struct drin_gemm_route {
  int32_t launches;
  int32_t family;
  int32_t bm, bn;
  int32_t w_planes, a_lo, f16, persist, indexed, accumulate;
  int32_t ksplit;
  int32_t splits;
  int64_t tiles;
  int64_t whole_tiles;
  int64_t tile0;
  int64_t work_items;
} drin_gemm_route;
typedef struct drin_gemm_probe_args {
  size_t struct_size;
  int32_t op;
  int32_t precision;
  int32_t accumulate;
  int32_t row_tile_wgs;
  int64_t row_tile_begin, row_tile_end;
  const void* a;
  const void* a_lo;
  int64_t lda;
  const void* b;
  const void* b_hi;
  const void* b_lo;
  int64_t ldb;
  const float* bias;
  void* y;
  int64_t ldy;
  int64_t rows;
  int32_t n_out, k;
  float* scratch;
  size_t scratch_floats;
  const int64_t* a_index;
  const float* row_scale;
  const float* b_scale;
  drin_gemm_route route;
} drin_gemm_probe_args;
DRIN_API int drin_gemm_probe(drin_gemm_probe_args* args, void* stream);

enum drin_wgrad_probe_op {
  DRIN_WGRAD_TN_GROUP = 1,
  DRIN_WGRAD_TN_F32_GROUP = 2,
  DRIN_WGRAD_TN = 3,
  DRIN_WGRAD_COLSUM_BATCH = 4,
  DRIN_WGRAD_PASS = 5,
  DRIN_WGRAD_NN = 6
};
enum drin_wgrad_kernel {
  DRIN_WGRAD_KERNEL_NONE = 0,
  DRIN_WGRAD_KERNEL_TN_BF16X3 = 1,
  DRIN_WGRAD_KERNEL_TN_F32_SMALL = 2,
  DRIN_WGRAD_KERNEL_TN_F32_LARGE = 3
};
enum drin_wgrad_wt_form { DRIN_WGRAD_WT_NONE = 0, DRIN_WGRAD_WT_F32_SCRATCH = 1, DRIN_WGRAD_WT_PLANES = 2 };
#define DRIN_WGRAD_PROBE_MAX 16
#define DRIN_WGRAD_ROUTE_LAUNCHES 8
typedef struct drin_wgrad_product {
  const float* dy;
  int64_t lddy;
  const float* x;
  int64_t ldx;
  const int64_t* x_index;
  float* dw;
  int64_t lddw;
  float* db;
  int64_t rows;
  int32_t n_out, k;
} drin_wgrad_product;
typedef struct drin_wgrad_product_route {
  int32_t kernel;
  int32_t slices;
  int32_t in_place;
  int32_t db_rode;
  int32_t db_slices;
  int32_t launch;
  int64_t rows_per_slice;
} drin_wgrad_product_route;
typedef struct drin_wgrad_route {
  int32_t gemm_launches;
  int32_t colsum_launches;
  int32_t sum_launches;
  int32_t reduce_launches;
  int32_t sum_dsts, sum_segs;
  int32_t nn_family;
  int32_t nn_bm, nn_bn, nn_splits, nn_wt_form, nn_accumulate;
  int64_t grid[DRIN_WGRAD_ROUTE_LAUNCHES];
  drin_wgrad_product_route product[DRIN_WGRAD_PROBE_MAX];
} drin_wgrad_route;
typedef struct drin_wgrad_probe_args {
  size_t struct_size;
  int32_t op;
  int32_t precision;
  int32_t staged;
  int32_t n_products;
  int32_t layers_done_after;
  int32_t accumulate;
  int32_t wt_form;
  int32_t reserved;
  float* scratch;
  size_t scratch_floats;
  float* wt;
  size_t wt_floats;
  drin_wgrad_product product[DRIN_WGRAD_PROBE_MAX];
  drin_wgrad_route route;
} drin_wgrad_probe_args;
DRIN_API int drin_wgrad_probe(drin_wgrad_probe_args* args, void* stream);

DRIN_API size_t drin_loss_workspace_bytes(int32_t batch);
DRIN_API int drin_triplet_topk(const float* scores, const uint8_t* answer, int32_t batch, int32_t num_candidates,
                               float margin, const int32_t* topk, int32_t num_topk, float* loss, float* d_scores,
                               int64_t* correct, void* workspace, size_t workspace_bytes, void* stream);

DRIN_API int drin_adam_step(float* param, const float* grad, float* exp_avg, float* exp_avg_sq, int64_t n,
                            float lerp_weight, float beta2, float one_minus_beta2, float bias_correction2_sqrt, float eps,
                            float neg_step_size, void* stream);

typedef struct {
  int32_t batch;
  int32_t num_candidates;
  int32_t embed_dim;
  int32_t image_dim;
  int32_t mention_tokens;
  int32_t image_regions;
  int32_t precision;
  float cosine_eps;
  float thres_tmim;
  float thres_imie;
} drin_melhi_config;

typedef struct {
  const float* mention_feature;
  const int64_t* mention_mask;
  const int64_t* start;
  const int64_t* end;
  const float* mention_image;
  const float* entity_feature;
  const float* entity_image;
} drin_melhi_batch;

typedef struct {
  const float *w_image_map_text, *b_image_map_text;
  const float *w_ih, *w_hh, *b_ih, *b_hh;
  const float *w_mention_final_map, *b_mention_final_map;
  const float *w_entity_final_map, *b_entity_final_map;
} drin_melhi_params;

typedef struct {
  float *w_image_map_text, *b_image_map_text;
  float *w_ih, *w_hh, *b_ih, *b_hh;
  float *w_mention_final_map, *b_mention_final_map;
  float *w_entity_final_map, *b_entity_final_map;
} drin_melhi_param_grads;

DRIN_API size_t drin_melhi_workspace_bytes(const drin_melhi_config* cfg, int for_training);

DRIN_API int drin_melhi_forward(const drin_melhi_config* cfg, const drin_melhi_batch* batch, const drin_melhi_params* params,
                                const int32_t* order, const int32_t* lengths, void* workspace, size_t workspace_bytes,
                                float* scores, void* stream);
DRIN_API int drin_melhi_backward(const drin_melhi_config* cfg, const drin_melhi_batch* batch, const drin_melhi_params* params,
                                 const int32_t* order, const int32_t* lengths, void* workspace, size_t workspace_bytes,
                                 const float* grad_scores, const drin_melhi_param_grads* grads, void* stream);

typedef struct {
  int32_t batch;
  int32_t num_candidates;
  int32_t embed_dim;
  int32_t image_dim;
  int32_t mention_tokens;
  int32_t image_regions;
  int32_t num_heads;
  int32_t entity_tokens;
  int32_t precision;
  float layer_norm_eps;
  float cosine_eps;
} drin_ghmfc_config;

typedef struct {
  const float* mention_feature;
  const int64_t* mention_mask;
  const float* mention_image;
  const float* entity_feature;
  const int64_t* entity_mask;
} drin_ghmfc_batch;

typedef struct {
  const float *a2b_wq, *a2b_wk, *a2b_wv;
  const float *a2b_in_bias;
  const float *a2b_wo, *a2b_bo;
  const float *a2b_ffn_w, *a2b_ffn_b;
  const float *b2a_in_w, *b2a_in_bias;
  const float *b2a_wo, *b2a_bo;
  const float *b2a_ffn_w, *b2a_ffn_b;
  const float *ln0_w, *ln0_b, *ln1_w, *ln1_b, *ln2_w, *ln2_b, *ln3_w, *ln3_b;
} drin_ghmfc_cross_params;

typedef struct {
  drin_ghmfc_cross_params t2v;
  drin_ghmfc_cross_params v2t;
  const float *w_text_linear, *b_text_linear;
  const float *w_image_linear, *b_image_linear;
  const float *w_score_linear, *b_score_linear;
  const float *w_entity, *b_entity;
} drin_ghmfc_params;

DRIN_API size_t drin_ghmfc_workspace_bytes(const drin_ghmfc_config* cfg);

DRIN_API int drin_ghmfc_forward(const drin_ghmfc_config* cfg, const drin_ghmfc_batch* batch, const drin_ghmfc_params* params,
                                void* workspace, size_t workspace_bytes, float* scores, float* mention_repr, void* stream);

DRIN_API int drin_attention(const float* q, int64_t ldq, const float* k, int64_t ldk, const float* v, int64_t ldv,
                            const int64_t* key_mask, float* out, int64_t ldo, int32_t batch, int32_t num_heads, int32_t q_len,
                            int32_t k_len, int32_t head_dim, void* stream);

DRIN_API int drin_attention_train_fwd(const float* q, int64_t ldq, const float* k, int64_t ldk, const float* v, int64_t ldv,
                                      const int64_t* key_mask, float* out, int64_t ldo, float* lse, int32_t batch,
                                      int32_t num_heads, int32_t q_len, int32_t k_len, int32_t head_dim, void* stream);

DRIN_API int drin_attention_bwd(const float* q, int64_t ldq, const float* k, int64_t ldk, const float* v, int64_t ldv,
                                const int64_t* key_mask, const float* out, int64_t ldo, const float* lse, const float* dout,
                                int64_t lddo, float* dq, int64_t lddq, float* dk, int64_t lddk, float* dv, int64_t lddv,
                                float* delta_scratch, int32_t batch, int32_t num_heads, int32_t q_len, int32_t k_len,
                                int32_t head_dim, void* stream);


DRIN_API int drin_attention_dropout_fwd(const float* q, int64_t ldq, const float* k, int64_t ldk, const float* v, int64_t ldv,
                                        const int64_t* key_mask, float* out, int64_t ldo, float* lse, int32_t batch,
                                        int32_t num_heads, int32_t q_len, int32_t k_len, int32_t head_dim, float p, uint64_t seed,
                                        uint64_t call, void* stream);
DRIN_API int drin_attention_dropout_bwd(const float* q, int64_t ldq, const float* k, int64_t ldk, const float* v, int64_t ldv,
                                        const int64_t* key_mask, const float* out, int64_t ldo, const float* lse,
                                        const float* dout, int64_t lddo, float* dq, int64_t lddq, float* dk, int64_t lddk,
                                        float* dv, int64_t lddv, float* delta_scratch, int32_t batch, int32_t num_heads,
                                        int32_t q_len, int32_t k_len, int32_t head_dim, float p, uint64_t seed, uint64_t call,
                                        void* stream);
DRIN_API int drin_attention_dropout_keep(uint64_t seed, uint64_t call, int32_t batch, int32_t num_heads, int32_t q_len,
                                         int32_t k_len, float p, uint8_t* keep_host);


DRIN_API int drin_attention_mfma_fwd(const float* q, int64_t ldq, const float* k, int64_t ldk, const float* v, int64_t ldv,
                                     const int64_t* key_mask, float* out, int64_t ldo, float* lse, int32_t batch,
                                     int32_t num_heads, int32_t q_len, int32_t k_len, int32_t head_dim, float p, uint64_t seed,
                                     uint64_t call, void* stream);
DRIN_API int drin_attention_mfma_bwd(const float* q, int64_t ldq, const float* k, int64_t ldk, const float* v, int64_t ldv,
                                     const int64_t* key_mask, const float* out, int64_t ldo, const float* lse, const float* dout,
                                     int64_t lddo, float* dq, int64_t lddq, float* dk, int64_t lddk, float* dv, int64_t lddv,
                                     float* delta_scratch, int32_t batch, int32_t num_heads, int32_t q_len, int32_t k_len,
                                     int32_t head_dim, float p, uint64_t seed, uint64_t call, void* stream);


DRIN_API int drin_layernorm_res_train_fwd(const float* x, const float* res, const float* gamma, const float* beta, float* y,
                                          float* mean, float* rstd, int64_t rows, int32_t width, float eps, void* stream);
DRIN_API size_t drin_layernorm_res_bwd_scratch_floats(int64_t rows, int32_t width);
DRIN_API int drin_layernorm_res_bwd(const float* x, const float* res, const float* mean, const float* rstd, const float* gamma,
                                    const float* dy, float* dh, float* dgamma, float* dbeta, float* scratch,
                                    size_t scratch_floats, int64_t rows, int32_t width, void* stream);

DRIN_API int drin_seq_max_train_fwd(const float* x, float* out, int32_t* idx, int32_t batch, int32_t seq_len, int32_t width,
                                    void* stream);
DRIN_API int drin_seq_max_bwd(const float* dout, const int32_t* idx, float* dx, int32_t batch, int32_t seq_len, int32_t width,
                              void* stream);

DRIN_API int drin_gate_mix_fwd(const float* tl, const float* vl, const float* ws, const float* bs, float* out, int32_t batch,
                               int32_t width, void* stream);
DRIN_API size_t drin_gate_mix_bwd_scratch_floats(int32_t batch, int32_t width);
DRIN_API int drin_gate_mix_bwd(const float* tl, const float* vl, const float* ws, const float* bs, const float* dout, float* dtl,
                               float* dvl, float* dws, float* dbs, float* scratch, size_t scratch_floats, int32_t batch,
                               int32_t width, void* stream);

DRIN_API int drin_cosine_rows_fwd(const float* x, const float* y, float* out, int32_t batch, int32_t num_candidates, int32_t width,
                                  float eps, void* stream);
DRIN_API int drin_cosine_rows_bwd(const float* x, const float* y, const float* dout, float* dx, float* dy, float* scratch,
                                  size_t scratch_floats, int32_t batch, int32_t num_candidates, int32_t width, float eps,
                                  void* stream);
DRIN_API int drin_entity_token_mean(const float* feat, const int64_t* mask, float* out, int64_t pairs, int32_t tokens,
                                    int32_t width, void* stream);


typedef enum {
  DRIN_ROW_ACT_NONE = 0,
  DRIN_ROW_ACT_RELU = 1,
  DRIN_ROW_ACT_GELU = 2
} drin_row_activation;

DRIN_API int drin_act_dropout_fwd(const float* x, float* y, int64_t rows, int32_t width, int32_t act, float p, uint64_t seed,
                                  uint64_t call, void* stream);
DRIN_API int drin_act_dropout_bwd(const float* x, const float* dy, float* dx, int64_t rows, int32_t width, int32_t act, float p,
                                  uint64_t seed, uint64_t call, void* stream);

DRIN_API int drin_span_mean_fwd(const float* seq, const int64_t* start, const int64_t* end, float* out, int32_t batch,
                                int32_t seq_len, int32_t width, void* stream);
DRIN_API int drin_span_mean_bwd(const float* dout, const int64_t* start, const int64_t* end, float* dseq, int32_t batch,
                                int32_t seq_len, int32_t width, void* stream);


typedef enum {
  DRIN_KC_GEMM = 0,
  DRIN_KC_POOL = 1,
  DRIN_KC_EDGE = 2,
  DRIN_KC_GCN = 3,
  DRIN_KC_STREAM = 4,
  DRIN_KC_GEMM_X3 = 5,
  DRIN_KC_GEMM_PLANES = 6,
  DRIN_KC_OPTIM = 7,
  DRIN_KC_LSTM = 8,
  DRIN_KC_CELL = 9,
  DRIN_KC_ATTN = 10,
  DRIN_KC_NORM = 11,
  DRIN_KC_COUNT = 12
} drin_kernel_class;

DRIN_API int drin_profile_begin(int max_launches);
DRIN_API int drin_profile_end(double* ms_by_class, int64_t* launches_by_class);
DRIN_API const char* drin_kernel_class_name(int kernel_class);

#ifdef __cplusplus
}
#endif
#endif
```

Before: 28.36 million pairs/s.

## Fold entity stream sums into pair layer and fuse mention vertex update

For non-IF16 precisions, the separate entity-stream reduction, the two entity projection GEMMs, mention_input1 and the layer-1 mention GEMM are removed. The pair layer-1 kernel now also accumulates e-weighted sums of h_text/h_image plus the edge-weight sums. A new mention-vertices kernel combines these with precomputed bias projections (wb_t, wb_i) to form vm1 and agg2 directly, and one 3B-row GEMM against W_h2 replaces the separate mention layer-2 path, followed by a bias+layernorm kernel. This cuts several small launches and GEMMs, at the cost of extra per-pair accumulation and LDS traffic in the pair kernel. It also lowers the side-permille knob and adds a layout self-check API.

```diff
diff --git a/drin_amd/_lib.py b/drin_amd/_lib.py
--- a/drin_amd/_lib.py
+++ b/drin_amd/_lib.py
@@ -194,6 +194,7 @@
     "drin_indexed_supported": (C.c_int, [C.POINTER(DrinConfigC)]),
     "drin_prepared_bytes": (C.c_size_t, [C.POINTER(DrinConfigC)]),
     "drin_fused_workspace_bytes": (C.c_size_t, [C.POINTER(DrinConfigC)]),
+    "drin_fused_layout_selfcheck": (C.c_int, [C.POINTER(DrinConfigC)]),
     "drin_workgroups_per_mention": (C.c_int32, [C.POINTER(DrinConfigC), C.c_int32]),
     "drin_index_status": (C.c_int, [C.c_void_p, C.c_void_p]),
     "drin_image_contraction_passes": (C.c_int32, [C.POINTER(DrinConfigC), C.c_int32]),
diff --git a/drin_amd/csrc/fused.h b/drin_amd/csrc/fused.h
--- a/drin_amd/csrc/fused.h
+++ b/drin_amd/csrc/fused.h
@@ -15,6 +15,7 @@
   size_t p_wmt, p_wmi, p_wcat1, p_ecat, p_wet, p_wei, p_wh1;
   size_t p_cimg_f16;
   size_t cimg_f16_scale;
+  size_t wb_t, wb_i;
   void build(const drin_config& c) {
     const size_t D = c.embed_dim, R = c.image_dim;
     Arena A;
@@ -40,6 +41,8 @@
     p_wh1 = A.take(D * D);
     p_cimg_f16 = A.take(D * R / 2 + 2);
     cimg_f16_scale = A.take(2);
+    wb_t = A.take(D);
+    wb_i = A.take(D);
     total = A.total;
   }
 };
@@ -99,6 +102,7 @@
   void* et1_lo;
   float* s2_part;
   int B, N, D4, chunks, ldhm;
+  int sums1;
   int act_v;
   float ln_eps;
 };
@@ -149,6 +153,23 @@
                           hipStream_t st);
 int launch_pair_final(const FinalArgs& a, hipStream_t st);
 
+struct MentionArgs {
+  const float* part;
+  const float* hm;
+  const float* wb_t;
+  const float* wb_i;
+  const float* b_h1;
+  const float* gamma;
+  const float* beta;
+  float* out;
+  int B, N, D4, chunks, ldhm;
+  int act_v;
+  float ln_eps;
+};
+int launch_mention_vertices(const MentionArgs& a, hipStream_t st);
+int launch_bias_layernorm_act(const float* h, const float* bias, const float* gamma, const float* beta, float* y, int64_t rows, int D,
+                              float eps, int act, hipStream_t st);
+
 struct GemmScratch {
   float* p = nullptr;
   size_t floats = 0;
diff --git a/drin_amd/csrc/fused_forward.hip b/drin_amd/csrc/fused_forward.hip
--- a/drin_amd/csrc/fused_forward.hip
+++ b/drin_amd/csrc/fused_forward.hip
@@ -12,6 +12,7 @@
   size_t span_mean, mimg, vm0, hmfu, q, e0m, e1m, xt, s_part, s_text, s_img, sig, tm, tm2, agg1, vm1, hm2, h_text, h_image,
       et1, s2_part, agg2, mt2, p_xt, p_xi, p_et1, xi_scale, splitk, splitk_floats, pair_splitk, pair_splitk_floats, total;
   int chunks;
+  static bool stream_sums(const drin_config& c) { return c.precision == DRIN_PREC_BF16X3_IF16; }
   void build(const drin_config& c) {
     const size_t B = c.batch, N = c.num_candidates, D = c.embed_dim, R = c.image_dim, M = B * N;
     chunks = (int)(B >= 2048 ? (N + 127) / 128 : B >= 1024 ? (N + 47) / 48 : (N + 15) / 16);
@@ -24,27 +25,29 @@
     e0m = A.take(4 * M);
     e1m = A.take(4 * M);
     xt = A.take(c.entity_tokens > 0 ? M * D : 0);
-    s_part = A.take(B * chunks * (2 * D + 2 * R + 4));
-    s_text = A.take(2 * B * D);
-    s_img = A.take(2 * B * R);
-    sig = A.take(4 * B);
-    tm = A.take(2 * B * D);
-    tm2 = A.take(2 * B * D);
-    agg1 = A.take(2 * B * D);
-    vm1 = A.take(2 * B * D);
-    hm2 = A.take(2 * B * D);
+    const size_t ss = stream_sums(c) ? 1 : 0;
+    s_part = A.take(ss * B * chunks * (2 * D + 2 * R + 4));
+    s_text = A.take(ss * 2 * B * D);
+    s_img = A.take(ss * 2 * B * R);
+    sig = A.take(ss * 4 * B);
+    tm = A.take(ss * 2 * B * D);
+    tm2 = A.take(ss * 2 * B * D);
+    agg1 = A.take(ss * 2 * B * D);
+    vm1 = A.take(3 * B * D);
+    agg2 = vm1 + 2 * B * D;
+    hm2 = A.take(3 * B * D);
+    mt2 = hm2 + 2 * B * D;
     h_text = A.take(M * D);
     h_image = A.take(M * D);
     et1 = A.take(M * D);
-    s2_part = A.take(B * chunks * 2 * D);
-    agg2 = A.take(B * D);
-    mt2 = A.take(B * D);
+    s2_part = A.take(B * chunks * (4 * D + 4));
     const bool planes = c.precision == DRIN_PREC_BF16X3 || c.precision == DRIN_PREC_BF16X3_ALL || c.precision == DRIN_PREC_BF16X3_IF16;
     p_xt = A.take(planes ? M * D : 0);
     p_xi = A.take(!planes ? 0 : c.num_entities > 0 ? M * R : c.precision == DRIN_PREC_BF16X3_IF16 ? M * R / 2 : 0);
     p_et1 = A.take(planes ? M * D : 0);
     xi_scale = A.take(c.precision == DRIN_PREC_BF16X3_IF16 ? M : 0);
     splitk_floats = 2 * B <= (size_t)kSmallSplitkMaxRows ? small_splitk_floats(2 * B, D + R) : 0;
+    if (3 * B <= (size_t)kSmallSplitkMaxRows && splitk_floats < small_splitk_floats(3 * B, D)) splitk_floats = small_splitk_floats(3 * B, D);
     if (planes && splitk_floats < tail_split_floor_floats()) splitk_floats = tail_split_floor_floats();
     splitk = A.take(splitk_floats);
     pair_splitk_floats = planes ? drin::pair_splitk_floats(M, D) : 0;
@@ -57,14 +60,15 @@
   const size_t B = c.batch, M = B * c.num_candidates, D = c.embed_dim, R = c.image_dim;
   FusedLayout L;
   L.build(c);
-  const size_t ch = (size_t)L.chunks, planes = c.precision != DRIN_PREC_F32;
+  const size_t ch = (size_t)L.chunks, planes = c.precision != DRIN_PREC_F32, ss = FusedLayout::stream_sums(c) ? 1 : 0;
   const Region ws[] = {
       {"span_mean", L.span_mean, B * D}, {"mimg", L.mimg, B * R}, {"vm0", L.vm0, 2 * B * D}, {"hmfu", L.hmfu, 4 * B * D},
       {"q", L.q, 2 * B * (D + R)}, {"e0m", L.e0m, 4 * M}, {"e1m", L.e1m, 4 * M}, {"xt", L.xt, c.entity_tokens > 0 ? M * D : 0},
-      {"s_part", L.s_part, B * ch * (2 * D + 2 * R + 4)}, {"s_text", L.s_text, 2 * B * D}, {"s_img", L.s_img, 2 * B * R},
-      {"sig", L.sig, 4 * B}, {"tm", L.tm, 2 * B * D}, {"tm2", L.tm2, 2 * B * D}, {"agg1", L.agg1, 2 * B * D}, {"vm1", L.vm1, 2 * B * D},
-      {"hm2", L.hm2, 2 * B * D}, {"h_text", L.h_text, M * D}, {"h_image", L.h_image, M * D}, {"et1", L.et1, M * D},
-      {"s2_part", L.s2_part, B * ch * 2 * D}, {"agg2", L.agg2, B * D}, {"mt2", L.mt2, B * D}, {"p_xt", L.p_xt, planes * M * D},
+      {"s_part", L.s_part, ss * B * ch * (2 * D + 2 * R + 4)}, {"s_text", L.s_text, ss * 2 * B * D}, {"s_img", L.s_img, ss * 2 * B * R},
+      {"sig", L.sig, ss * 4 * B}, {"tm", L.tm, ss * 2 * B * D}, {"tm2", L.tm2, ss * 2 * B * D}, {"agg1", L.agg1, ss * 2 * B * D},
+      {"vm1", L.vm1, 3 * B * D}, {"hm2", L.hm2, 3 * B * D},
+      {"h_text", L.h_text, M * D}, {"h_image", L.h_image, M * D}, {"et1", L.et1, M * D},
+      {"s2_part", L.s2_part, B * ch * (4 * D + 4)}, {"p_xt", L.p_xt, planes * M * D},
       {"p_xi", L.p_xi, !planes ? 0 : c.num_entities > 0 ? M * R : c.precision == DRIN_PREC_BF16X3_IF16 ? M * R / 2 : 0},
       {"p_et1", L.p_et1, planes * M * D}, {"xi_scale", L.xi_scale, c.precision == DRIN_PREC_BF16X3_IF16 ? M : 0},
       {"splitk", L.splitk, L.splitk_floats}, {"pair_splitk", L.pair_splitk, L.pair_splitk_floats}};
@@ -76,7 +80,8 @@
       {"k_t", P.k_t, D}, {"k_i", P.k_i, D}, {"c_txt", P.c_txt, D * D}, {"c_img", P.c_img, D * R}, {"cb_t", P.cb_t, D}, {"cb_i", P.cb_i, D},
       {"p_ctxt", P.p_ctxt, D * D}, {"p_cimg", P.p_cimg, D * R}, {"p_wh2", P.p_wh2, D * D}, {"p_wmt", P.p_wmt, D * D},
       {"p_wmi", P.p_wmi, D * R}, {"p_wcat1", P.p_wcat1, 2 * D * D}, {"p_ecat", P.p_ecat, D * (D + R)}, {"p_wet", P.p_wet, D * D},
-      {"p_wei", P.p_wei, D * R}, {"p_wh1", P.p_wh1, D * D}, {"p_cimg_f16", P.p_cimg_f16, D * R / 2}, {"cimg_f16_scale", P.cimg_f16_scale, 2}};
+      {"p_wei", P.p_wei, D * R}, {"p_wh1", P.p_wh1, D * D}, {"p_cimg_f16", P.p_cimg_f16, D * R / 2}, {"cimg_f16_scale", P.cimg_f16_scale, 2},
+      {"wb_t", P.wb_t, D}, {"wb_i", P.wb_i, D}};
   return regions_hold("Prepared", pr, (int)(sizeof(pr) / sizeof(pr[0])), P.total);
 }
 
@@ -91,7 +96,7 @@
 #define DRIN_SIDE_WGS 64
 #endif
 #ifndef DRIN_SIDE_PERMILLE
-#define DRIN_SIDE_PERMILLE 900
+#define DRIN_SIDE_PERMILLE 800
 #endif
 #ifndef DRIN_SIDE_MIN_TILES
 #define DRIN_SIDE_MIN_TILES 1200
@@ -245,6 +250,8 @@
   DRIN_TRY(launch_gemm_nn(L1.w_h, D, params->w_entity_image, R, pb + P.c_img, R, D, R, D, false, F32, st));
   DRIN_TRY(launch_gemm_nt(params->b_entity_text, D, L1.w_h, D, L1.b_h, pb + P.cb_t, D, 1, D, D, false, F32, st));
   DRIN_TRY(launch_gemm_nt(params->b_entity_image, D, L1.w_h, D, L1.b_h, pb + P.cb_i, D, 1, D, D, false, F32, st));
+  DRIN_TRY(launch_gemm_nt(params->b_entity_text, D, L1.w_h, D, nullptr, pb + P.wb_t, D, 1, D, D, false, F32, st));
+  DRIN_TRY(launch_gemm_nt(params->b_entity_image, D, L1.w_h, D, nullptr, pb + P.wb_i, D, 1, D, D, false, F32, st));
   {
     const size_t dd = (size_t)D * D, dr = (size_t)D * R;
     __bf16* q = reinterpret_cast<__bf16*>(pb + P.p_ctxt);
@@ -301,17 +308,12 @@
                         sk.floats, weight_planes ? pb + P.p_wh2 : nullptr);
 }
 
-int run_folded_tail(const drin_config* cfg, const drin_params* params, const float* pb, const Prepared& P, int chunks,
-                    const float* s2_part, const float* vm1, float* agg2, float* mt2, const float* hm2, const float* e1m, float* h2,
-                    const float* et1, const void* et1_hi, bool weight_planes, GemmScratch sk, GemmScratch pair_sk, float* scores,
-                    hipStream_t st) {
+static int folded_tail_pairs(const drin_config* cfg, const drin_params* params, const float* pb, const Prepared& P, int chunks,
+                             const float* mt2, const float* hm2, const float* e1m, float* h2, const float* et1, const void* et1_hi,
+                             GemmScratch pair_sk, float* scores, hipStream_t st) {
   const int B = cfg->batch, N = cfg->num_candidates, D = cfg->embed_dim, prec = folded_precision(cfg);
   const int64_t M = (int64_t)B * N;
   const drin_layer_params& L2 = params->layer[1];
-  DRIN_TRY(launch_mention_input2(s2_part, vm1, agg2, B, D, N, chunks, st));
-  DRIN_TRY(launch_gemm_nt(agg2, D, L2.w_h, D, L2.b_h, mt2, D, B, D, D, false, prec, st, sk.p, sk.floats,
-                          weight_planes ? pb + P.p_wh2 : nullptr));
-  DRIN_TRY(launch_layernorm_gelu(mt2, L2.ln_weight, L2.ln_bias, mt2, nullptr, nullptr, B, D, cfg->layer_norm_eps, st, vertex_act(cfg)));
   if (et1_hi) {
     const __bf16* e1 = static_cast<const __bf16*>(et1_hi);
     const __bf16* w2 = reinterpret_cast<const __bf16*>(pb + P.p_wh2);
@@ -333,6 +335,19 @@
   fa.chunks = chunks;
   fa.cos_eps = cfg->cosine_eps;
   return launch_pair_final(fa, st);
+}
+
+int run_folded_tail(const drin_config* cfg, const drin_params* params, const float* pb, const Prepared& P, int chunks,
+                    const float* s2_part, const float* vm1, float* agg2, float* mt2, const float* hm2, const float* e1m, float* h2,
+                    const float* et1, const void* et1_hi, bool weight_planes, GemmScratch sk, GemmScratch pair_sk, float* scores,
+                    hipStream_t st) {
+  const int B = cfg->batch, N = cfg->num_candidates, D = cfg->embed_dim, prec = folded_precision(cfg);
+  const drin_layer_params& L2 = params->layer[1];
+  DRIN_TRY(launch_mention_input2(s2_part, vm1, agg2, B, D, N, chunks, st));
+  DRIN_TRY(launch_gemm_nt(agg2, D, L2.w_h, D, L2.b_h, mt2, D, B, D, D, false, prec, st, sk.p, sk.floats,
+                          weight_planes ? pb + P.p_wh2 : nullptr));
+  DRIN_TRY(launch_layernorm_gelu(mt2, L2.ln_weight, L2.ln_bias, mt2, nullptr, nullptr, B, D, cfg->layer_norm_eps, st, vertex_act(cfg)));
+  return folded_tail_pairs(cfg, params, pb, P, chunks, mt2, hm2, e1m, h2, et1, et1_hi, pair_sk, scores, st);
 }
 
 static int forward_prepared_on_stream(const drin_config* cfg, const drin_batch* b, const drin_params* params, const void* prepared,
@@ -450,25 +465,29 @@
   sa.xi_f16 = if16 ? static_cast<void*>(xi_hi) : nullptr;
   sa.e0m = ws + L.e0m;
   sa.e1m = ws + L.e1m;
-  sa.s_part = ws + L.s_part;
   sa.T = cfg->entity_tokens;
   sa.Ke = cfg->entity_objects;
   sa.chunks = L.chunks;
   sa.bf16_features = bf16_feat ? 1 : 0;
-  sa.s_text = ws + L.s_text;
-  sa.s_img = ws + L.s_img;
-  sa.sig = ws + L.sig;
+  if (if16) {
+    sa.s_part = ws + L.s_part;
+    sa.s_text = ws + L.s_text;
+    sa.s_img = ws + L.s_img;
+    sa.sig = ws + L.sig;
+  }
   DRIN_TRY(launch_entity_stream(sa, st));
-  if (L.chunks > 1)
-    DRIN_TRY(launch_reduce_stream_partials(ws + L.s_part, ws + L.s_text, ws + L.s_img, ws + L.sig, B, D, R, L.chunks, st));
-  DRIN_TRY(launch_gemm_nt_pair({ws + L.s_text, params->w_entity_text, nullptr, ws + L.tm, D, D, D, 2 * (int64_t)B, D, D, wp(P.p_wet)},
-                               {ws + L.s_img, params->w_entity_image, nullptr, ws + L.tm2, R, R, D, 2 * (int64_t)B, D, R,
-                                wp(P.p_wei)},
-                               prec, st, msk.p, msk.floats));
-  DRIN_TRY(launch_mention_input1(ws + L.tm, ws + L.tm2, ws + L.sig, params->b_entity_text, params->b_entity_image, vm0, ws + L.agg1, B, D, N, st));
   float* vm1 = ws + L.vm1;
-  DRIN_TRY(launch_gemm_nt(ws + L.agg1, D, L1.w_h, D, L1.b_h, vm1, D, 2 * (int64_t)B, D, D, false, prec, st, msk.p, msk.floats, wp(P.p_wh1)));
-  DRIN_TRY(run_folded_mention_finish(cfg, params, pb, P, planes, vm1, ws + L.hm2, msk, st));
+  if (if16) {
+    if (L.chunks > 1)
+      DRIN_TRY(launch_reduce_stream_partials(ws + L.s_part, ws + L.s_text, ws + L.s_img, ws + L.sig, B, D, R, L.chunks, st));
+    DRIN_TRY(launch_gemm_nt_pair({ws + L.s_text, params->w_entity_text, nullptr, ws + L.tm, D, D, D, 2 * (int64_t)B, D, D, wp(P.p_wet)},
+                                 {ws + L.s_img, params->w_entity_image, nullptr, ws + L.tm2, R, R, D, 2 * (int64_t)B, D, R,
+                                  wp(P.p_wei)},
+                                 prec, st, msk.p, msk.floats));
+    DRIN_TRY(launch_mention_input1(ws + L.tm, ws + L.tm2, ws + L.sig, params->b_entity_text, params->b_entity_image, vm0, ws + L.agg1, B, D, N, st));
+    DRIN_TRY(launch_gemm_nt(ws + L.agg1, D, L1.w_h, D, L1.b_h, vm1, D, 2 * (int64_t)B, D, D, false, prec, st, msk.p, msk.floats, wp(P.p_wh1)));
+    DRIN_TRY(run_folded_mention_finish(cfg, params, pb, P, planes, vm1, ws + L.hm2, msk, st));
+  }
   if (planes) {
     const __bf16* ct = reinterpret_cast<const __bf16*>(pb + P.p_ctxt);
     const __bf16* ci = reinterpret_cast<const __bf16*>(pb + P.p_cimg);
@@ -513,9 +532,30 @@
   }
   pa.s2_part = ws + L.s2_part;
   pa.chunks = L.chunks;
+  pa.sums1 = if16 ? 0 : 1;
   DRIN_TRY(launch_pair_layer1(pa, st));
-  return run_folded_tail(cfg, params, pb, P, L.chunks, ws + L.s2_part, vm1, ws + L.agg2, ws + L.mt2, ws + L.hm2, ws + L.e1m, ws + L.h_text,
-                         planes ? nullptr : ws + L.et1, planes ? e1_hi : nullptr, planes, msk, psk, scores, st);
+  if (if16)
+    return run_folded_tail(cfg, params, pb, P, L.chunks, ws + L.s2_part, vm1, ws + L.agg2, ws + L.mt2, ws + L.hm2, ws + L.e1m, ws + L.h_text,
+                           planes ? nullptr : ws + L.et1, planes ? e1_hi : nullptr, planes, msk, psk, scores, st);
+  MentionArgs ma;
+  memset(&ma, 0, sizeof(ma));
+  ma.part = ws + L.s2_part;
+  ma.hm = hmfu;
+  ma.ldhm = 2 * D;
+  ma.wb_t = pb + P.wb_t;
+  ma.wb_i = pb + P.wb_i;
+  ma.b_h1 = L1.b_h;
+  ma.gamma = L1.ln_weight;
+  ma.beta = L1.ln_bias;
+  ma.out = vm1;
+  ma.B = B, ma.N = N, ma.D4 = D / 4, ma.chunks = L.chunks;
+  ma.act_v = vertex_act(cfg), ma.ln_eps = cfg->layer_norm_eps;
+  DRIN_TRY(launch_mention_vertices(ma, st));
+  const drin_layer_params& L2 = params->layer[1];
+  DRIN_TRY(launch_gemm_nt(vm1, D, L2.w_h, D, nullptr, ws + L.hm2, D, 3 * (int64_t)B, D, D, false, prec, st, msk.p, msk.floats, wp(P.p_wh2)));
+  DRIN_TRY(launch_bias_layernorm_act(ws + L.mt2, L2.b_h, L2.ln_weight, L2.ln_bias, ws + L.mt2, B, D, cfg->layer_norm_eps, vertex_act(cfg), st));
+  return folded_tail_pairs(cfg, params, pb, P, L.chunks, ws + L.mt2, ws + L.hm2, ws + L.e1m, ws + L.h_text, planes ? nullptr : ws + L.et1,
+                           planes ? e1_hi : nullptr, psk, scores, st);
 }
 
 }
@@ -561,6 +601,12 @@
   return DRIN_E_INDEX;
 }
 
+int drin_fused_layout_selfcheck(const drin_config* cfg) {
+  DRIN_TRY(validate_config(cfg));
+  DRIN_TRY(fused_supported(cfg));
+  return fused_layout_selfcheck(*cfg);
+}
+
 size_t drin_fused_workspace_bytes(const drin_config* cfg) {
   if (validate_config(cfg) != DRIN_OK || fused_supported(cfg) != DRIN_OK) return 0;
   FusedLayout L;
diff --git a/drin_amd/csrc/fused_kernels.hip b/drin_amd/csrc/fused_kernels.hip
--- a/drin_amd/csrc/fused_kernels.hip
+++ b/drin_amd/csrc/fused_kernels.hip
@@ -20,10 +20,12 @@
     else
       return load_row_stream<RV>(row, (int)(threadIdx.x & 63), R4);
   };
+  constexpr bool SUMS = XSCALE;
+  constexpr bool FLAT = TOKENS && sizeof(FT) == 2 && EXACT && DV == 3;
   float* l_mobj = lds;
   float* l_q = l_mobj + a.Km * R;
   float* l_red = l_q + 2 * R;
-  float* l_mt = l_red + 2 * D + 2 * R;
+  float* l_mt = l_red + (SUMS ? 2 * D + 2 * R : FLAT ? 4 * 768 : 0);
   float* l_small = l_mt + 3 * D;
   const int wave = threadIdx.x >> 6, lane = threadIdx.x & 63;
   const int64_t b = blockIdx.y;
@@ -94,7 +96,6 @@
       if (stop < 0) stop += T;
       stop = stop < 0 ? 0 : (stop > T ? T : stop);
       const FT* base = f_text + e * (int64_t)T * D;
-      constexpr bool FLAT = sizeof(FT) == 2 && EXACT && DV == 3;
       const Row<DV> cls = load_row_stream<DV>(base, lane, D4);
       Row<DV> acc = zero_row<DV>();
       int t = 1;
@@ -158,6 +159,19 @@
             for (int j = 0; j < DV; ++j) acc.v[j] = acc.v[j] + r[u].v[j];
         }
       }
+#ifdef DRIN_STREAM_ROWS8
+      if constexpr (sizeof(FT) == 4 && EXACT && DV == 3 && !XSCALE) {
+        for (; t + 8 <= stop; t += 8) {
+          Row<DV> r[8];
+#pragma unroll
+          for (int u = 0; u < 8; ++u) r[u] = load_row_stream<DV>(base + (int64_t)(t + u) * D, lane, D4);
+#pragma unroll
+          for (int u = 0; u < 8; ++u)
+#pragma unroll
+            for (int j = 0; j < DV; ++j) acc.v[j] = acc.v[j] + r[u].v[j];
+        }
+      }
+#endif
       for (; t + 4 <= stop; t += 4) {
         const Row<DV> r0 = load_row_stream<DV>(base + (int64_t)t * D, lane, D4);
         const Row<DV> r1 = load_row_stream<DV>(base + (int64_t)(t + 1) * D, lane, D4);
@@ -233,15 +247,18 @@
       a.e1m[2 * M + p] = n_it * a.mask[2];
       a.e1m[3 * M + p] = n_ii * a.mask[3];
     }
-    axpy_row<DV>(S_tt, e_tt, xt);
-    axpy_row<DV>(S_it, e_it, xt);
-    axpy_row<RV>(S_ti, e_ti, xi);
-    axpy_row<RV>(S_ii, e_ii, xi);
-    sg_tt += e_tt;
-    sg_ti += e_ti;
-    sg_it += e_it;
-    sg_ii += e_ii;
-  }
+    if constexpr (SUMS) {
+      axpy_row<DV>(S_tt, e_tt, xt);
+      axpy_row<DV>(S_it, e_it, xt);
+      axpy_row<RV>(S_ti, e_ti, xi);
+      axpy_row<RV>(S_ii, e_ii, xi);
+      sg_tt += e_tt;
+      sg_ti += e_ti;
+      sg_it += e_it;
+      sg_ii += e_ii;
+    }
+  }
+  if constexpr (!SUMS) return;
 
   for (int w = 0; w < 4; ++w) {
     __syncthreads();
@@ -295,7 +312,13 @@
 
 size_t entity_stream_lds_bytes(const StreamArgs& a) {
   const size_t D = (size_t)a.D4 * 4, R = (size_t)a.R4 * 4;
-  return sizeof(float) * (a.Km * R + 2 * R + 2 * D + 2 * R + 3 * D + a.Km + 4);
+  const bool sums = a.xi_scale != nullptr;
+  const bool flat = a.bf16_features && a.T > 0 && a.D4 == 192 && a.R4 == 512;
+  size_t pad = 0;
+#ifdef DRIN_STREAM_LDS_PAD
+  pad = DRIN_STREAM_LDS_PAD;
+#endif
+  return pad + sizeof(float) * (a.Km * R + 2 * R + (sums ? 2 * D + 2 * R : flat ? 4 * 768 : 0) + 3 * D + a.Km + 4);
 }
 
 template <int DV, int RV, bool TOKENS, bool EXACT, typename FT, bool XSCALE = false>
@@ -435,7 +458,7 @@
 
 template <int DV, bool EXACT, bool GENERIC_ACT = false>
 __global__ void __launch_bounds__(256) k_pair_layer1(const PairArgs a) {
-  __shared__ __attribute__((aligned(16))) float l_red[2 * DV * 256];
+  __shared__ __attribute__((aligned(16))) float l_red[4 * DV * 256 + 4];
   __shared__ __attribute__((aligned(16))) float l_const[6 * DV * 256];
   const int D4 = EXACT ? DV * 64 : a.D4, D = D4 * 4;
   const int wave = threadIdx.x >> 6, lane = threadIdx.x & 63;
@@ -454,11 +477,25 @@
   const float *l_hm_t = l_const, *l_hm_i = l_const + LD, *l_ct = l_const + 2 * LD, *l_ci = l_const + 3 * LD;
   const float *l_gamma = l_const + 4 * LD, *l_beta = l_const + 5 * LD;
   Row<DV> S_t = zero_row<DV>(), S_i = zero_row<DV>();
+  Row<DV> A_t = zero_row<DV>(), A_i = zero_row<DV>();
+  float sg_tt = 0.f, sg_ti = 0.f, sg_it = 0.f, sg_ii = 0.f;
+  const bool sums1 = a.sums1 != 0;
   for (int n = n_begin + wave; n < n_end; n += 4) {
+    __asm__ volatile("" ::: "memory");
     const int64_t p = b * a.N + n;
     const Row<DV> ht = load_row_stream<DV>(a.h_text + p * D, lane, D4);
     const Row<DV> hi = load_row_stream<DV>(a.h_image + p * D, lane, D4);
     const float e_tt = a.e0m[p], e_ti = a.e0m[M + p], e_it = a.e0m[2 * M + p], e_ii = a.e0m[3 * M + p];
+    if (sums1) {
+      axpy_row_pk<DV>(A_t, e_tt, ht);
+      axpy_row_pk<DV>(A_t, e_ti, hi);
+      axpy_row_pk<DV>(A_i, e_it, ht);
+      axpy_row_pk<DV>(A_i, e_ii, hi);
+      sg_tt += e_tt;
+      sg_ti += e_ti;
+      sg_it += e_it;
+      sg_ii += e_ii;
+    }
     const Row<DV> et1 = ln_gelu_row_lds<DV, GENERIC_ACT>(combine_rows_lds<DV>(ht, e_tt, l_hm_t, e_it, l_hm_i, l_ct, lane, D4),
                                                          l_gamma, l_beta, lane, D4, a.ln_eps, a.act_v);
     if (a.et1) store_row<DV>(a.et1 + p * D, et1, lane, D4);
@@ -477,15 +514,30 @@
         float* p1 = l_red + DV * 256 + (j * 64 + lane) * 4;
         st4(p0, w == 0 ? S_t.v[j] : ld4(p0) + S_t.v[j]);
         st4(p1, w == 0 ? S_i.v[j] : ld4(p1) + S_i.v[j]);
+        if (sums1) {
+          float* p2 = l_red + 2 * DV * 256 + (j * 64 + lane) * 4;
+          float* p3 = l_red + 3 * DV * 256 + (j * 64 + lane) * 4;
+          st4(p2, w == 0 ? A_t.v[j] : ld4(p2) + A_t.v[j]);
+          st4(p3, w == 0 ? A_i.v[j] : ld4(p3) + A_i.v[j]);
+        }
+      }
+      if (sums1 && lane == 0) {
+        float* s4 = l_red + 4 * DV * 256;
+        s4[0] = (w == 0 ? 0.f : s4[0]) + sg_tt;
+        s4[1] = (w == 0 ? 0.f : s4[1]) + sg_ti;
+        s4[2] = (w == 0 ? 0.f : s4[2]) + sg_it;
+        s4[3] = (w == 0 ? 0.f : s4[3]) + sg_ii;
       }
     }
   }
   __syncthreads();
-  float* out = a.s2_part + (b * a.chunks + blockIdx.x) * (int64_t)(2 * D);
-  for (int i = threadIdx.x; i < 2 * D4; i += 256) {
+  const int rows = sums1 ? 4 : 2;
+  float* out = a.s2_part + (b * a.chunks + blockIdx.x) * (int64_t)(sums1 ? 4 * D + 4 : 2 * D);
+  for (int i = threadIdx.x; i < rows * D4; i += 256) {
     const int which = i / D4, c4 = i - which * D4;
     st4(out + which * D + c4 * 4, ld4(l_red + which * DV * 256 + c4 * 4));
   }
+  if (sums1 && threadIdx.x < 4) out[4 * D + threadIdx.x] = l_red[4 * DV * 256 + threadIdx.x];
 }
 
 int launch_pair_layer1(const PairArgs& a, hipStream_t st) {
@@ -509,6 +561,100 @@
   return DRIN_OK;
 }
 
+template <int DV, bool GENERIC_ACT>
+__global__ void __launch_bounds__(256) k_mention_vertices(const MentionArgs a) {
+  const int wave = threadIdx.x >> 6, lane = threadIdx.x & 63;
+  const int64_t b = (int64_t)blockIdx.x * 4 + wave;
+  if (b >= a.B) return;
+  const int D4 = a.D4, D = D4 * 4, width = 4 * D + 4;
+  const float inv_n = 1.0f / (float)a.N;
+  Row<DV> S2_t = zero_row<DV>(), S2_i = zero_row<DV>(), A_t = zero_row<DV>(), A_i = zero_row<DV>();
+  float4 sg = make_float4(0.f, 0.f, 0.f, 0.f);
+  for (int c = 0; c < a.chunks; ++c) {
+    const float* p = a.part + (b * a.chunks + c) * (int64_t)width;
+    const Row<DV> r0 = load_row<DV>(p, lane, D4), r1 = load_row<DV>(p + D, lane, D4);
+    const Row<DV> r2 = load_row<DV>(p + 2 * D, lane, D4), r3 = load_row<DV>(p + 3 * D, lane, D4);
+#pragma unroll
+    for (int j = 0; j < DV; ++j) {
+      S2_t.v[j] = S2_t.v[j] + r0.v[j];
+      S2_i.v[j] = S2_i.v[j] + r1.v[j];
+      A_t.v[j] = A_t.v[j] + r2.v[j];
+      A_i.v[j] = A_i.v[j] + r3.v[j];
+    }
+    sg = sg + ld4(p + 4 * D);
+  }
+  const Row<DV> wb_t = load_row<DV>(a.wb_t, lane, D4), wb_i = load_row<DV>(a.wb_i, lane, D4), b_h1 = load_row<DV>(a.b_h1, lane, D4);
+  auto vertex = [&](const Row<DV>& A, float sa, float sb, const float* hm) -> Row<DV> {
+    const Row<DV> h = load_row<DV>(hm, lane, D4);
+    Row<DV> x;
+#pragma unroll
+    for (int j = 0; j < DV; ++j) x.v[j] = fma4(sb, wb_i.v[j], fma4(sa, wb_t.v[j], A.v[j])) * inv_n + (h.v[j] + b_h1.v[j]);
+    return ln_gelu_row_lds<DV, GENERIC_ACT>(x, a.gamma, a.beta, lane, D4, a.ln_eps, a.act_v);
+  };
+  const Row<DV> vm1_t = vertex(A_t, sg.x, sg.y, a.hm + b * a.ldhm);
+  const Row<DV> vm1_i = vertex(A_i, sg.z, sg.w, a.hm + ((int64_t)a.B + b) * a.ldhm);
+  Row<DV> agg2;
+#pragma unroll
+  for (int j = 0; j < DV; ++j) agg2.v[j] = (S2_t.v[j] * inv_n + S2_i.v[j] * inv_n) + vm1_t.v[j];
+  store_row<DV>(a.out + b * D, vm1_t, lane, D4);
+  store_row<DV>(a.out + ((int64_t)a.B + b) * D, vm1_i, lane, D4);
+  store_row<DV>(a.out + (2 * (int64_t)a.B + b) * D, agg2, lane, D4);
+}
+
+int launch_mention_vertices(const MentionArgs& a, hipStream_t st) {
+  if (a.B <= 0) return DRIN_OK;
+  KernelTimer timer(DRIN_KC_GCN, st);
+  const dim3 grid((unsigned)cdiv(a.B, 4));
+  const bool generic = a.act_v != DRIN_ACT_GELU;
+  if (a.D4 <= 64) {
+    if (generic) hipLaunchKernelGGL((k_mention_vertices<1, true>), grid, dim3(256), 0, st, a);
+    else hipLaunchKernelGGL((k_mention_vertices<1, false>), grid, dim3(256), 0, st, a);
+  } else if (a.D4 <= 192) {
+    if (generic) hipLaunchKernelGGL((k_mention_vertices<3, true>), grid, dim3(256), 0, st, a);
+    else hipLaunchKernelGGL((k_mention_vertices<3, false>), grid, dim3(256), 0, st, a);
+  } else {
+    set_error("mention_vertices: D=%d outside the built instantiations", a.D4 * 4);
+    return DRIN_E_UNSUPPORTED;
+  }
+  DRIN_CHECK_LAUNCH("k_mention_vertices");
+  return DRIN_OK;
+}
+
+template <int DV, bool GENERIC_ACT>
+__global__ void __launch_bounds__(256) k_bias_layernorm_act(const float* h, const float* __restrict__ bias,
+                                                            const float* __restrict__ gamma, const float* __restrict__ beta,
+                                                            float* y, int64_t rows, int D4, float eps, int act) {
+  const int wave = threadIdx.x >> 6, lane = threadIdx.x & 63;
+  const int64_t r = (int64_t)blockIdx.x * 4 + wave;
+  if (r >= rows) return;
+  Row<DV> x = load_row<DV>(h + r * D4 * 4, lane, D4);
+  const Row<DV> bb = load_row<DV>(bias, lane, D4);
+#pragma unroll
+  for (int j = 0; j < DV; ++j) x.v[j] = x.v[j] + bb.v[j];
+  store_row<DV>(y + r * D4 * 4, ln_gelu_row_lds<DV, GENERIC_ACT>(x, gamma, beta, lane, D4, eps, act), lane, D4);
+}
+
+int launch_bias_layernorm_act(const float* h, const float* bias, const float* gamma, const float* beta, float* y, int64_t rows, int D,
+                              float eps, int act, hipStream_t st) {
+  if (rows <= 0) return DRIN_OK;
+  KernelTimer timer(DRIN_KC_GCN, st);
+  const dim3 grid((unsigned)cdiv(rows, (int64_t)4));
+  const bool generic = act != DRIN_ACT_GELU;
+  const int D4 = D / 4;
+  if (D4 <= 64) {
+    if (generic) hipLaunchKernelGGL((k_bias_layernorm_act<1, true>), grid, dim3(256), 0, st, h, bias, gamma, beta, y, rows, D4, eps, act);
+    else hipLaunchKernelGGL((k_bias_layernorm_act<1, false>), grid, dim3(256), 0, st, h, bias, gamma, beta, y, rows, D4, eps, act);
+  } else if (D4 <= 192) {
+    if (generic) hipLaunchKernelGGL((k_bias_layernorm_act<3, true>), grid, dim3(256), 0, st, h, bias, gamma, beta, y, rows, D4, eps, act);
+    else hipLaunchKernelGGL((k_bias_layernorm_act<3, false>), grid, dim3(256), 0, st, h, bias, gamma, beta, y, rows, D4, eps, act);
+  } else {
+    set_error("bias_layernorm_act: D=%d outside the built instantiations", D);
+    return DRIN_E_UNSUPPORTED;
+  }
+  DRIN_CHECK_LAUNCH("k_bias_layernorm_act");
+  return DRIN_OK;
+}
+
 __global__ void __launch_bounds__(256) k_mention_input2(const float* __restrict__ part, const float* __restrict__ mt1,
                                                         float* __restrict__ out, int D, int chunks, float inv_n) {
   const int64_t b = blockIdx.y;
diff --git a/include/drin_hip.h b/include/drin_hip.h
--- a/include/drin_hip.h
+++ b/include/drin_hip.h
@@ -193,6 +193,8 @@
                                    const void* prepared, void* workspace, size_t workspace_bytes, float* scores,
                                    void* stream);
 DRIN_API int32_t drin_workgroups_per_mention(const drin_config* cfg, int32_t cached);
+
+DRIN_API int drin_fused_layout_selfcheck(const drin_config* cfg);
 
 DRIN_API int32_t drin_image_contraction_passes(const drin_config* cfg, int32_t indexed);
 
```

Result: slower. 27.78 million pairs/s (-2.1%).
